# GT-STAR-Lab/MARBLER

Hardware: AMD Instinct MI355X
Metric: env agent-steps/sec (higher is better)
Workload: dtype f32

## Files before the change

marbler_amd/csrc/probes/diag.h:

```cpp
#pragma once

#ifndef RG_CHUNK
#define RG_CHUNK 5
#endif
#ifndef RG_MAX_WAVES
#define RG_MAX_WAVES 1024
#endif
#ifndef RG_TPE_W4
#define RG_TPE_W4 3
#endif
#ifndef RG_TPE_W5
#define RG_TPE_W5 0
#endif
#ifndef RG_TPE_W78
#define RG_TPE_W78 1
#endif
#ifndef RG_TPE_NO_W3
#define RG_TPE_WAVES_ATTR(n) __attribute__((amdgpu_waves_per_eu(n)))
#else
#define RG_TPE_WAVES_ATTR(n)
#endif

namespace rg {
#ifdef RG_STAMPS
constexpr bool kStampsBuild = true;
#else
constexpr bool kStampsBuild = false;
#endif
#ifdef RG_HOST_SIM
constexpr bool kHostSim = true;
#else
constexpr bool kHostSim = false;
#endif
#ifdef RG_TPE_GUARD
constexpr bool kTpeGuard = true;
#else
constexpr bool kTpeGuard = false;
#endif
}

#ifdef RG_STAMPS
#define RG_STAMPS_BEGIN()                                                    \
    const unsigned long long t_start = __builtin_amdgcn_s_memtime();         \
    int stamps[8] = {0, 0, 0, 0, 0, 0, 0, 0};                                \
    RG_STAMPS_CLOCK_BEGIN()
#define RG_STAMP_ALWAYS_5() stamps[5] = static_cast<int>(__builtin_amdgcn_s_memtime() - t_start)
#define RG_PIN1(a) asm volatile("" ::"v"(a))
#define RG_PIN2(a, b) asm volatile("" ::"v"(a), "v"(b))
#define RG_PIN3(a, b, c) asm volatile("" ::"v"(a), "v"(b), "v"(c))
#define RG_PIN4(a, b, c, d) asm volatile("" ::"v"(a), "v"(b), "v"(c), "v"(d))
#define RG_PIN5(a, b, c, d, e) asm volatile("" ::"v"(a), "v"(b), "v"(c), "v"(d), "v"(e))
#ifdef RG_STAMPS_EPI
#define RG_STAMP(i) \
    if ((i) > 2) stamps[i] = static_cast<int>(__builtin_amdgcn_s_memtime() - t_start)
#define RG_STAMP_E(i) stamps[i] = static_cast<int>(__builtin_amdgcn_s_memtime() - t_start)
#else
#define RG_STAMP(i) stamps[i] = static_cast<int>(__builtin_amdgcn_s_memtime() - t_start)
#define RG_STAMP_E(i)
#endif
#ifdef RG_STAMPS_CLOCK
#define RG_STAMPS_CLOCK_BEGIN() const unsigned long long rt_start = __builtin_amdgcn_s_memrealtime();
#define RG_STAMPS_CLOCK_END() stamps[5] = static_cast<int>(__builtin_amdgcn_s_memrealtime() - rt_start);
#else
#define RG_STAMPS_CLOCK_BEGIN()
#define RG_STAMPS_CLOCK_END()
#endif
#define RG_STAMPS_WRITE(lane_, qp_, e0_, E_, max_sweeps_)                                     \
    RG_STAMPS_CLOCK_END()                                                                     \
    if ((lane_) == 0 && (qp_)) {                                                              \
        stamps[7] = (max_sweeps_);                                                            \
        for (int i_ = 0; i_ < 8; ++i_)                                                        \
            if ((e0_) + i_ < (E_)) (qp_)[(e0_) + i_] = stamps[i_];                            \
    }
#else
#define RG_STAMPS_BEGIN()
#define RG_STAMP_ALWAYS_5()
#define RG_PIN1(a)
#define RG_PIN2(a, b)
#define RG_PIN3(a, b, c)
#define RG_PIN4(a, b, c, d)
#define RG_PIN5(a, b, c, d, e)
#define RG_STAMP(i)
#define RG_STAMP_E(i)
#define RG_STAMPS_WRITE(lane_, qp_, e0_, E_, max_sweeps_)
#endif

#if defined(RG_STAMPS) && defined(RG_STAMPS_CTRL)
#define RG_CTRL_TICKS_PARAM , int *ctrl_ticks = nullptr
#define RG_CTRL_TICKS_ARG , ctrl_ticks
#define RG_CTRL_LOCALS() int ctrl_ticks[5] = {0, 0, 0, 0, 0};
#define RG_CTRL_BEGIN(x, y, c, s)                      \
    asm volatile("" ::"v"(x), "v"(y), "v"(c), "v"(s)); \
    unsigned long long ctrl_t = __builtin_amdgcn_s_memtime();
#define RG_CTRL_TICK(i)                                                     \
    {                                                                       \
        const unsigned long long t_ = __builtin_amdgcn_s_memtime();         \
        ctrl_ticks[i] += static_cast<int>(t_ - ctrl_t);                     \
        ctrl_t = t_;                                                        \
    }
#define RG_CTRL_PIN_ROUNDS(GW_, fx, bp, emax) \
    _Pragma("unroll") for (int r_ = 0; r_ < (GW_) - 1; ++r_) asm volatile("" ::"v"(fx[r_]), "v"(bp[r_]), "v"(emax[r_]));
#define RG_CTRL_PIN2(a, b) asm volatile("" ::"v"(a), "v"(b))
#define RG_CTRL_COUNT_SWEEPS(n) ctrl_ticks[3] += (n)
#define RG_HEADING_SINCOS(th, s, c)                                                   \
    asm volatile("" ::"v"(th));                                                       \
    const unsigned long long t_sc = __builtin_amdgcn_s_memtime();                     \
    sincos_spec(th, s, c);                                                            \
    asm volatile("" ::"v"(s), "v"(c));                                                \
    ctrl_ticks[4] += static_cast<int>(__builtin_amdgcn_s_memtime() - t_sc)
#define RG_CTRL_REPORT()                                                                                        \
    stamps[0] = ctrl_ticks[0];                                                                                  \
    stamps[1] = ctrl_ticks[1];                                                                                  \
    stamps[2] = ctrl_ticks[2] * 100 + ctrl_ticks[3];           \
    stamps[3] = ctrl_ticks[4];
#else
#define RG_CTRL_TICKS_PARAM
#define RG_CTRL_TICKS_ARG
#define RG_CTRL_LOCALS()
#define RG_CTRL_BEGIN(x, y, c, s)
#define RG_CTRL_TICK(i)
#define RG_CTRL_PIN_ROUNDS(GW_, fx, bp, emax)
#define RG_CTRL_PIN2(a, b)
#define RG_CTRL_COUNT_SWEEPS(n)
#define RG_HEADING_SINCOS(th, s, c) sincos_spec(th, s, c)
#define RG_CTRL_REPORT()
#endif

#if defined(RG_STAMPS) && defined(RG_STAMPS_CHUNK)
#define RG_CHUNK_LOCALS() int chunk_ticks[4] = {0, 0, 0, 0};
#define RG_CHUNK_DENSE_BEGIN() const unsigned long long t_dense0 = __builtin_amdgcn_s_memtime();
#define RG_CHUNK_DENSE_END(dmin)                                          \
    asm volatile("" ::"v"(dmin));                                         \
    const unsigned long long t_dense1 = __builtin_amdgcn_s_memtime();     \
    chunk_ticks[0] += static_cast<int>(t_dense1 - t_dense0);              \
    chunk_ticks[2] += 1;
#define RG_CHUNK_REPLAY_END(rx, ry)                                                    \
    asm volatile("" ::"v"(rx), "v"(ry));                                               \
    chunk_ticks[1] += static_cast<int>(__builtin_amdgcn_s_memtime() - t_dense1);       \
    chunk_ticks[3] += 1;
#define RG_CHUNK_REPORT()           \
    stamps[0] = chunk_ticks[0];     \
    stamps[1] = chunk_ticks[1];     \
    stamps[2] = chunk_ticks[2] * 1000 + chunk_ticks[3];
#else
#define RG_CHUNK_LOCALS()
#define RG_CHUNK_DENSE_BEGIN()
#define RG_CHUNK_DENSE_END(dmin)
#define RG_CHUNK_REPLAY_END(rx, ry)
#define RG_CHUNK_REPORT()
#endif

#if defined(RG_STAMPS) && !defined(RG_STAMPS_EPI)
#define RG_TSTAMP_MAIN(i) RG_STAMP(i)
#define RG_TSTAMP_EPI(i)
#define RG_TSTAMP_PERIOD(it0) \
    if ((it0) == 0) RG_STAMP(2)
#elif defined(RG_STAMPS)
#define RG_TSTAMP_MAIN(i)
#define RG_TSTAMP_EPI(i) RG_STAMP_E(i)
#define RG_TSTAMP_PERIOD(it0) \
    if ((it0) != 0) RG_STAMP_E(2)
#else
#define RG_TSTAMP_MAIN(i)
#define RG_TSTAMP_EPI(i)
#define RG_TSTAMP_PERIOD(it0)
#endif
#ifdef RG_STAMPS
#define RG_PIN_ARR1(N_, a) _Pragma("unroll") for (int i_ = 0; i_ < (N_); ++i_) asm volatile("" ::"v"(a[i_]))
#define RG_PIN_ARR2(N_, a, b) _Pragma("unroll") for (int i_ = 0; i_ < (N_); ++i_) asm volatile("" ::"v"(a[i_]), "v"(b[i_]))
#define RG_PIN_ARR3(N_, a, b, c) _Pragma("unroll") for (int i_ = 0; i_ < (N_); ++i_) asm volatile("" ::"v"(a[i_]), "v"(b[i_]), "v"(c[i_]))
#define RG_PIN_ARR5(N_, a, b, c, d, e) \
    _Pragma("unroll") for (int i_ = 0; i_ < (N_); ++i_) asm volatile("" ::"v"(a[i_]), "v"(b[i_]), "v"(c[i_]), "v"(d[i_]), "v"(e[i_]))
#else
#define RG_PIN_ARR1(N_, a)
#define RG_PIN_ARR2(N_, a, b)
#define RG_PIN_ARR3(N_, a, b, c)
#define RG_PIN_ARR5(N_, a, b, c, d, e)
#endif
#ifdef RG_TPE_DIAG
#define RG_TPE_DIAG_LOCALS() int diag = 0;
#define RG_TPE_DIAG_SWEEPS(sw, it0) diag |= (sw) << ((it0) == 0 ? 8 : 0)
#define RG_TPE_DIAG_REPLAY(it0, j0, CH_) diag |= 1 << (16 + ((it0) ? 3 : 0) + (j0) / (CH_))
#define RG_TPE_DIAG_REPORT(max_sweeps) max_sweeps = diag
#else
#define RG_TPE_DIAG_LOCALS()
#define RG_TPE_DIAG_SWEEPS(sw, it0)
#define RG_TPE_DIAG_REPLAY(it0, j0, CH_)
#define RG_TPE_DIAG_REPORT(max_sweeps)
#endif
#ifdef RG_TPE_GUARD
#define RG_GUARDED(dst, lo, hi, code, stmt) \
    if ((dst) < (lo) || (dst) >= (hi)) atomicOr(sg.flag, (code)); else { stmt; }
#else
#define RG_GUARDED(dst, lo, hi, code, stmt) stmt
#endif

#ifdef RG_IPM_STAMPS
namespace rg { namespace ipm { __device__ unsigned long long ipm_ticks[8]; } }
#define RG_IPM_T0() unsigned long long ipm_t_ = __builtin_amdgcn_s_memtime();
#define RG_IPM_TICK(i)                                                                              \
    {                                                                                               \
        const unsigned long long t2_ = __builtin_amdgcn_s_memtime();                                \
        if (threadIdx.x == 0 && blockIdx.x == 0) rg::ipm::ipm_ticks[i] += t2_ - ipm_t_;             \
        ipm_t_ = t2_;                                                                               \
    }
#else
#define RG_IPM_T0()
#define RG_IPM_TICK(i)
#endif
```

marbler_amd/csrc/step_group.h:

```cpp
#pragma once
#include <hip/hip_runtime.h>
#include <stdint.h>

#include <type_traits>

#include "device_common.h"
#include "ipm_qp.h"
#include "lidar.h"
#include "team.h"
#include "probes/diag.h"

namespace rg {

__device__ __forceinline__ void out_store4(float *p, float a, float b, float c, float d) {
    *reinterpret_cast<float4 *>(p) = make_float4(a, b, c, d);
}
__device__ __forceinline__ void out_store1(float *p, float a) {
    *p = a;
}

constexpr int CHUNK = RG_CHUNK;
static_assert(CHUNK >= 1 && CHUNK <= 5, "the sparse collision pre-test covers sub-steps 0..2 and 3..4 of a chunk: longer chunks would go untested");

template <int GW, int QPM = 0, typename QpLds = void, bool SPAN = false>
__device__ __forceinline__ int controller(const rg_scenario_params &p, const Consts &k, int N, int ag, bool lane_ok,
                                          bool upd, float x, float y, float c, float s, float gx, float gy, float &v,
                                          float &w, QpLds *qp RG_CTRL_TICKS_PARAM) {
    RG_CTRL_BEGIN(x, y, c, s)
    const float xix = x + k.pd * c, xiy = y + k.pd * s;
    float ux = gx - xix, uy = gy - xiy;
    {
        const float nrm = norm2_spec(ux, uy);
        const float sc = k.pvl / nrm;
        const bool clip = nrm > k.pvl;
        ux = clip ? ux * sc : ux;
        uy = clip ? uy * sc : uy;
    }
    if constexpr (QPM == RG_QP_CVXOPT) {
        {
            const float n2u = ux * ux + uy * uy;
            const bool clip = n2u > k.bml * k.bml;
            if (__any(clip)) {
                const float sc = k.bml / __builtin_sqrtf(n2u);
                ux = clip ? ux * sc : ux;
                uy = clip ? uy * sc : uy;
            }
        }
        const int lane_ = threadIdx.x;
        qp->rec[lane_] = make_float4(xix, xiy, ux, uy);
        __syncthreads();
        int iters = 0;
        if (upd) iters = ipm::solve_qp_n<GW>(N, ipm::make_consts(p), qp->rec + (lane_ & ~(GW - 1)), qp->ws[lane_ / GW], ag);
        __syncthreads();
        const float4 r = qp->rec[lane_];
        ux = r.z;
        uy = r.w;
        RG_CTRL_TICK(1);
        float vv = c * ux + s * uy;
        float ww = k.inv_pd * (-s * ux + c * uy);
        ww = ww > k.wlim ? k.wlim : ww;
        ww = ww < -k.wlim ? -k.wlim : ww;
        vv = vv > k.vmax ? k.vmax : vv;
        vv = vv < -k.vmax ? -k.vmax : vv;
        ww = ww > k.wmax ? k.wmax : ww;
        ww = ww < -k.wmax ? -k.wmax : ww;
        v = upd ? vv : v;
        w = upd ? ww : w;
        RG_CTRL_TICK(2);
        return iters;
    }
    const float bgain = p.barrier_gain, ugain = p.unsafe_barrier_gain, qp_rtol = p.qp_rtol;
    const int qp_cap = p.qp_max_sweeps;
    const bool has_unsafe = p.barrier_has_unsafe_gain != 0;
    float ex[GW - 1], ey[GW - 1], fx[GW - 1], fy[GW - 1], bp[GW - 1], emax[GW - 1];
    float mu[GW - 1], dmu[GW - 1];
    auto pair_consts = [&](float pxi, float pyi, int K, int i) {
        const float dx = xix - pxi, dy = xiy - pyi;
        const float ee = dx * dx + dy * dy;
        const float h = ee - k.r2;
        const float gain = ((h >= 0.0f) | !has_unsafe) ? bgain : ugain;
        const float b = gain * ((h * h) * h);
        const float n2 = 2.0f * ee;
        const bool ok = lane_ok & ((ag ^ K) < N) & (n2 > 0.0f);
        const float rn2 = ok ? 1.0f / n2 : 0.0f;
        ex[i] = dx;
        ey[i] = dy;
        fx[i] = dx * rn2;
        fy[i] = dy * rn2;
        bp[i] = (0.5f * b) * rn2;
        emax[i] = ok ? fmaxf(__builtin_fabsf(dx), __builtin_fabsf(dy)) : 0.0f;
    };
    const bool helper = SPAN && (threadIdx.x & GW) != 0;
    if constexpr (SPAN) {
        static_assert(GW == 8, "16-lane rows of two 8-lane halves");
        const float mx = mirror_upper_half(xix), my = mirror_upper_half(xiy);
        static_for<0, 4>([&](auto SS) {
            constexpr int S = decltype(SS)::value;
            const int K = helper ? S ^ 7 : S;
            if constexpr (S == 0) pair_consts(mx, my, K, 6);
            else pair_consts(xor_lane<S>(mx), xor_lane<S>(my), K, (S ^ 7) - 1);
        });
        static_for<1, 4>([&](auto SS) {
            constexpr int S = decltype(SS)::value, J = (S ^ 7) - 1;
            ex[S - 1] = ex[J];
            ey[S - 1] = ey[J];
            fx[S - 1] = fx[J];
            fy[S - 1] = fy[J];
            bp[S - 1] = bp[J];
            emax[S - 1] = emax[J];
        });
        static_for<3, 7>([&](auto JJ) {
            constexpr int J = decltype(JJ)::value;
            ex[J] = to_lower_half(ex[J]);
            ey[J] = to_lower_half(ey[J]);
            fx[J] = to_lower_half(fx[J]);
            fy[J] = to_lower_half(fy[J]);
            bp[J] = to_lower_half(bp[J]);
            emax[J] = to_lower_half(emax[J]);
        });
    } else {
        static_for<1, GW>([&](auto KK) {
            constexpr int K = decltype(KK)::value;
            pair_consts(xor_lane<K>(xix), xor_lane<K>(xiy), K, K - 1);
        });
    }
    static_for<0, GW - 1>([&](auto KK) { mu[decltype(KK)::value] = dmu[decltype(KK)::value] = 0.0f; });
    RG_CTRL_PIN_ROUNDS(GW, fx, bp, emax)
    RG_CTRL_TICK(0);
    {
        const float n2u = ux * ux + uy * uy;
        const bool clip = n2u > k.bml * k.bml;
        if (__any(clip)) {
            const float sc = k.bml / __builtin_sqrtf(n2u);
            ux = clip ? ux * sc : ux;
            uy = clip ? uy * sc : uy;
        }
    }
    const float uhx = ux, uhy = uy;
    bool active = upd & !helper;
    int sweeps = 0, my_sweeps = 0;
    auto sweep = [&](auto PH) {
        constexpr int PHASE = decltype(PH)::value;
        ++sweeps;
        if (active) {
            float chg = 0.0f, pa = 0.0f, pb = 0.0f;
            static_for<1, GW>([&](auto KK) {
                constexpr int K = decltype(KK)::value;
                const float pux = xor_lane<K>(ux), puy = xor_lane<K>(uy);
                const float c0 = mu[K - 1] - bp[K - 1];
                const float t = __builtin_fmaf(fy[K - 1], puy - uy, c0);
                float mn = __builtin_fmaf(fx[K - 1], pux - ux, t);
                mn = (mn > 0.0f) ? mn : 0.0f;
                const float delta = mn - mu[K - 1];
                mu[K - 1] = mn;
                ux = __builtin_fmaf(delta, ex[K - 1], ux);
                uy = __builtin_fmaf(delta, ey[K - 1], uy);
                chg = fmaxf(chg, __builtin_fabsf(delta) * emax[K - 1]);
                if constexpr (PHASE == 2) dmu[K - 1] = delta;
                if constexpr (PHASE == 3) {
                    const float dd = delta - dmu[K - 1];
                    pa = __builtin_fmaf(dd, delta, pa);
                    pb = __builtin_fmaf(dd, dd, pb);
                    dmu[K - 1] = delta;
                }
            });
            my_sweeps = sweeps;
            const float um = lane_ok ? fmaxf(__builtin_fabsf(ux), __builtin_fabsf(uy)) : 0.0f;
            const float gchg = group_max_nonneg<GW>(chg);
            const float gum = fmaxf(k.bml, group_max_nonneg<GW>(um));
            active = (gchg > qp_rtol * gum) & (sweeps < qp_cap);
            if constexpr (PHASE == 3) {
                if (active) {
                    const float ga = group_sum<GW>(pa), gb = group_sum<GW>(pb);
                    const bool ok = (gb > 0.0f) & (ga < 0.0f) & (-ga < 32.0f * gb);
                    const float gam = ok ? ga / gb : 0.0f;
                    float sx = uhx, sy = uhy;
                    static_for<1, GW>([&](auto KK) {
                        constexpr int K = decltype(KK)::value;
                        float m = __builtin_fmaf(-gam, dmu[K - 1], mu[K - 1]);
                        m = (m > 0.0f) ? m : 0.0f;
                        mu[K - 1] = m;
                        sx = __builtin_fmaf(m, ex[K - 1], sx);
                        sy = __builtin_fmaf(m, ey[K - 1], sy);
                    });
                    ux = sx;
                    uy = sy;
                }
            }
        }
    };
    while (__any(active)) {
        sweep(std::integral_constant<int, 1>{});
        if (!__any(active)) break;
        sweep(std::integral_constant<int, 2>{});
        if (!__any(active)) break;
        sweep(std::integral_constant<int, 3>{});
        if (!__any(active)) break;
        sweep(std::integral_constant<int, 0>{});
    }
    if constexpr (SPAN) {
        ux = to_upper_half(ux);
        uy = to_upper_half(uy);
    }
    RG_CTRL_PIN2(ux, uy);
    RG_CTRL_TICK(1);
    float vv = c * ux + s * uy;
    float ww = k.inv_pd * (-s * ux + c * uy);
    ww = ww > k.wlim ? k.wlim : ww;
    ww = ww < -k.wlim ? -k.wlim : ww;
    vv = vv > k.vmax ? k.vmax : vv;
    vv = vv < -k.vmax ? -k.vmax : vv;
    ww = ww > k.wmax ? k.wmax : ww;
    ww = ww < -k.wmax ? -k.wmax : ww;
    v = upd ? vv : v;
    w = upd ? ww : w;
    RG_CTRL_PIN2(v, w);
    RG_CTRL_COUNT_SWEEPS(sweeps);
    RG_CTRL_TICK(2);
    return my_sweeps;
}

template <int GW, int OD, int NT>
__device__ __forceinline__ void write_neighbour_obs(Lds<GW> &lds, int N, int Knb, int ag, int gbase, bool lane_ok,
                                                    float x, float y, float *obs_row) {
    constexpr int M = NT > 0 ? NT - 1 : GW - 1;
    unsigned long long key[M > 0 ? M : 1];
    bool ok[M > 0 ? M : 1];
    int rank[M > 0 ? M : 1], who[M > 0 ? M : 1];
    static_for<0, M>([&](auto RR) {
        constexpr int r = decltype(RR)::value;
        int j = ag + r + 1;
        j = j >= N ? j - N : j;
        j = j & (GW - 1);
        who[r] = j;
        const float2 pxy = *reinterpret_cast<const float2 *>(&lds.own[gbase + j][0]);
        const float dx = pxy.x - x, dy = pxy.y - y;
        const float d2 = dx * dx + dy * dy;
        ok[r] = lane_ok & (r + 1 < N);
        const unsigned int hi = ok[r] ? __builtin_bit_cast(unsigned int, d2) : 0xFFFFFFFFu;
        key[r] = (static_cast<unsigned long long>(hi) << 32) | static_cast<unsigned int>(j);
        rank[r] = M - 1 - r;
    });
    const bool all_others = Knb >= N - 1;
    static_for<1, M>([&](auto KK) {
        constexpr int k = decltype(KK)::value;
        static_for<0, k>([&](auto QQ) {
            constexpr int q = decltype(QQ)::value;
            const int q_first = key[q] < key[k] ? 1 : 0;
            rank[k] += q_first;
            rank[q] -= q_first;
        });
    });
    float row[M > 0 ? M : 1][OD];
    static_for<0, M>([&](auto RR) {
        constexpr int r = decltype(RR)::value;
        const float *src = &lds.own[gbase + who[r]][0];
        if constexpr (OD == 4) {
            const float4 v = *reinterpret_cast<const float4 *>(src);
            row[r][0] = v.x;
            row[r][1] = v.y;
            row[r][2] = v.z;
            row[r][3] = v.w;
        } else {
#pragma unroll
            for (int c = 0; c < OD; ++c) row[r][c] = src[c];
        }
    });
    static_for<0, M>([&](auto RR) {
        constexpr int r = decltype(RR)::value;
        const int j = who[r];
        const int slot = all_others ? (j < ag ? j : j - 1) : rank[r];
        if (ok[r] & (all_others | (slot < Knb))) {
            float *o = obs_row + (slot + 1) * OD;
            if constexpr (OD == 4) {
                out_store4(o, row[r][0], row[r][1], row[r][2], row[r][3]);
            } else {
#pragma unroll
                for (int c = 0; c < OD; ++c) o[c] = row[r][c];
            }
        }
    });
}

template <int SCN, int GW, bool OBS_ONLY, int NT, bool AHEAD, bool GYM, int QPM = 0, typename QpLds = void, typename Sync = WgSync,
          bool LIDAR = false, bool TEAM = false, bool SPAN = false>
__device__ __forceinline__ void step_once(const KernelArgs &a, Lds<GW> &lds, const StepView &sv, QpLds *qp_lds = nullptr,
                                          const rg_lidar_params *lid = nullptr, const rg_team_params *tm = nullptr) {
    static_assert(!SPAN || (GW == 8 && QPM == 0 && !GYM && !LIDAR && !TEAM), "the 16-lane rows: exact mode, GW = 8, no side blocks");
    constexpr int RW = SPAN ? 2 * GW : GW;
    constexpr int EPW = WAVE / RW;
    RG_STAMPS_BEGIN()
    const rg_scenario_params &p = a.p;
    const Consts &k = a.k;
    const float *q_poses = a.st.poses, *q_carry = a.st.carry_dist, *q_ret = a.st.ep_return, *q_sum = a.st.done_return_sum;
    const int32_t *q_steps = a.st.episode_steps, *q_act = sv.actions, *q_cnt = a.st.done_count, *q_stp = a.st.done_steps_sum;
    int32_t *q_el = GYM ? sv.io.elapsed : nullptr;
    const int q_tl = GYM ? sv.io.time_limit : 0;
    const int32_t *q_rc = a.st.reset_count, *q_nep = AHEAD ? a.st.next_episode : nullptr;
    const float *q_nin = AHEAD ? a.st.next_init : nullptr;
    const int q_nst = AHEAD ? a.next_stride : 0;
    const int q_E = a.E, q_epw = a.envs_per_wave, q_P = p.num_prey, q_N = p.n_agents, q_G = gridDim.x;
    asm volatile("" ::"s"(q_poses), "s"(q_carry), "s"(q_ret), "s"(q_sum), "s"(q_steps), "s"(q_act), "s"(q_cnt), "s"(q_stp),
                 "s"(q_E), "s"(q_epw), "s"(q_P), "s"(q_N), "s"(q_G), "s"(q_rc));
    if constexpr (GYM) asm volatile("" ::"s"(q_el), "s"(q_tl));
    if constexpr (AHEAD) asm volatile("" ::"s"(q_nep), "s"(q_nin), "s"(q_nst));
    const float *q_prey = a.st.prey_loc;
    const uint8_t *q_sen = a.st.prey_sensed, *q_cap = a.st.prey_captured, *q_loaded = a.st.loaded, *q_grid = a.st.grid;
    const uint8_t *q_pix = a.st.pixel_type, *q_reached = a.st.reached_goal;
    const int32_t *q_gcol = a.st.goal_col, *q_msg = a.st.messages, *q_zone = a.st.zone_load, *q_load = a.st.load;
    if constexpr (SCN == RG_SCN_PREDATOR_CAPTURE_PREY) asm volatile("" ::"s"(q_prey), "s"(q_sen), "s"(q_cap));
    else if constexpr (SCN == RG_SCN_WAREHOUSE) asm volatile("" ::"s"(q_loaded));
    else if constexpr (SCN == RG_SCN_SIMPLE) asm volatile("" ::"s"(q_prey));
    else if constexpr (SCN == RG_SCN_ARCTIC_TRANSPORT) asm volatile("" ::"s"(q_grid), "s"(q_pix), "s"(q_reached), "s"(q_gcol));
    else asm volatile("" ::"s"(q_msg), "s"(q_zone), "s"(q_load));
    int32_t *q_tidx = TEAM ? tm->team_index : nullptr;
    const float *q_tstep = TEAM ? tm->agent_step : nullptr, *q_tsr = TEAM ? tm->sensing_radius : nullptr;
    const float *q_tcr = TEAM ? tm->capture_radius : nullptr;
    const int32_t *q_ttq = TEAM ? tm->torque : nullptr;
    const int q_tC = TEAM ? tm->n_sets : 1;
    if constexpr (TEAM) {
        asm volatile("" ::"s"(q_tidx), "s"(q_tstep), "s"(q_tC));
        if constexpr (SCN == RG_SCN_PREDATOR_CAPTURE_PREY) asm volatile("" ::"s"(q_tsr), "s"(q_tcr));
        else if constexpr (SCN == RG_SCN_MATERIAL_TRANSPORT) asm volatile("" ::"s"(q_ttq));
    }

    const int N = NT > 0 ? NT : q_N;
    const int lane = threadIdx.x;
    const int ag = lane & (GW - 1);
    const int g = lane / RW;
    const int gbase = lane & ~(RW - 1);
    const bool helper = SPAN && (lane & GW) != 0;
    const int epw = q_epw > 0 ? q_epw : EPW;
    const int chunk = xcd_chunk(q_G);
    const int e = chunk * epw + g;
    const bool env_ok = (g < epw) & (e < q_E);
    const bool lane_ok = env_ok && ag < N;
    const bool env_st = env_ok & !helper, lane_st = lane_ok & !helper;
    const size_t eN = static_cast<size_t>(e) * N;

#define RG_LATE(v) asm volatile("" : "+v"(v))
    float x = 0.0f, y = 0.0f, th = 0.0f, carry = 0.0f;
    int act = 4;
    int steps_raw = 0;
    float agent_step = 0.0f, sr = 0.0f, cr = 0.0f;
    float st_ret = 0.0f, st_sum = 0.0f;
    int st_cnt = 0, st_steps = 0;
    const bool stats = (!OBS_ONLY) && q_ret != nullptr;
    int pix = 0, reached = 0;
    int team_raw = 0, tq_raw = 0;
    if constexpr (TEAM) {
        if (env_ok) team_raw = q_tidx[e];
    }
    if (lane_ok) {
        const float *X = q_poses + eN * 3;
        x = X[ag];
        y = X[N + ag];
        th = X[2 * N + ag];
        if constexpr (!OBS_ONLY) act = q_act[eN + ag];
        if constexpr (SCN == RG_SCN_ARCTIC_TRANSPORT) pix = q_pix[eN + ag];
        if constexpr (!TEAM) {
        agent_step = p.agent_step[ag];
        if constexpr (SCN == RG_SCN_PREDATOR_CAPTURE_PREY) {
            sr = p.sensing_radius[ag];
            cr = p.capture_radius[ag];
        }
        }
        if constexpr (!OBS_ONLY) carry = q_carry[eN + ag];
        if constexpr (TEAM) {
            const size_t ti = static_cast<size_t>(team_clamp(team_raw, q_tC)) * N + ag;
            agent_step = q_tstep[ti];
            if constexpr (SCN == RG_SCN_PREDATOR_CAPTURE_PREY) {
                sr = q_tsr[ti];
                cr = q_tcr[ti];
            }
            if constexpr (SCN == RG_SCN_MATERIAL_TRANSPORT) tq_raw = q_ttq[ti];
        }
    }
    int rc_raw = -1;
    const bool ahead = AHEAD && (!OBS_ONLY) && q_nst > 0 && a.auto_reset;
    int nx_tag = -2;
    float nx_pose[3] = {0.0f, 0.0f, 0.0f};
    float nx_a = 0.0f, nx_b = 0.0f;
    uint32_t nx_grid[7] = {0, 0, 0, 0, 0, 0, 0};
    auto load_next = [&](bool want) {
        if (want) {
            const float *nb = q_nin + static_cast<size_t>(e) * q_nst;
            if (ag < N) {
                nx_pose[0] = nb[ag];
                nx_pose[1] = nb[N + ag];
                nx_pose[2] = nb[2 * N + ag];
            }
            if constexpr (SCN == RG_SCN_PREDATOR_CAPTURE_PREY || SCN == RG_SCN_SIMPLE) {
                if (ag < q_P) {
                    nx_a = nb[3 * N + 2 * ag];
                    nx_b = nb[3 * N + 2 * ag + 1];
                }
            } else if constexpr (SCN == RG_SCN_MATERIAL_TRANSPORT) {
                if (ag < 2) nx_a = nb[3 * N + ag];
            } else if constexpr (SCN == RG_SCN_ARCTIC_TRANSPORT) {
                const uint32_t *gb = reinterpret_cast<const uint32_t *>(nb + 3 * N);
#pragma unroll
                for (int t = 0; t < 6; ++t) nx_grid[t] = gb[ag * 6 + t];
                nx_grid[6] = gb[24];
            }
        }
    };
    int el_raw = 0;
    if (env_ok) {
        steps_raw = q_steps[e];
        if (!OBS_ONLY && a.auto_reset) rc_raw = q_rc[e];
        if constexpr (GYM) el_raw = q_el[e];
        if (ahead) nx_tag = q_nep[e];
        if (stats && ag == 0) {
            st_ret = q_ret[e];
            st_sum = q_sum[e];
            st_cnt = q_cnt[e];
            st_steps = q_stp[e];
        }
    }
    uint32_t sen_lo = 0, sen_hi = 0, cap_lo = 0, cap_hi = 0;
    int flag_raw[4] = {0, 0, 0, 0};
    int loaded = 0;
    float goal_x = 0.0f, goal_y = 0.0f;
    uint32_t grid_pre[6] = {0, 0, 0, 0, 0, 0};
    int goal_col = 1;
    int load = 0, zone0 = 0, zone1 = 0;
    int msg[4] = {0, 0, 0, 0};
    float2 prey_r[8];
#pragma unroll
    for (int t = 0; t < 8; ++t) prey_r[t] = make_float2(0.0f, 0.0f);
    static_assert(SCN != RG_SCN_ARCTIC_TRANSPORT || GW == 4, "ArcticTransport is a 4-agent scenario");
    if constexpr (SCN == RG_SCN_PREDATOR_CAPTURE_PREY) {
        const int P = q_P;
        if (P <= 8) {
            if (env_ok) {
                const float2 *src = reinterpret_cast<const float2 *>(q_prey) + static_cast<size_t>(e) * P;
#pragma unroll
                for (int t = 0; t < 8; ++t) prey_r[t] = src[t < P ? t : P - 1];
                if (ag < P) {
                    flag_raw[0] = q_sen[static_cast<size_t>(e) * P + ag];
                    flag_raw[1] = q_cap[static_cast<size_t>(e) * P + ag];
                }
                if constexpr (GW < 8)
                    if (ag + GW < P) {
                        flag_raw[2] = q_sen[static_cast<size_t>(e) * P + ag + GW];
                        flag_raw[3] = q_cap[static_cast<size_t>(e) * P + ag + GW];
                    }
            }
        } else {
            if (env_ok) {
                for (int i = ag; i < 2 * P; i += GW) lds.prey[g][i] = q_prey[static_cast<size_t>(e) * 2 * P + i];
                for (int i = ag; i < P; i += GW) {
                    const uint32_t sb = q_sen[static_cast<size_t>(e) * P + i] != 0;
                    const uint32_t cb = q_cap[static_cast<size_t>(e) * P + i] != 0;
                    if (i < 32) {
                        sen_lo |= sb << i;
                        cap_lo |= cb << i;
                    } else {
                        sen_hi |= sb << (i - 32);
                        cap_hi |= cb << (i - 32);
                    }
                }
            }
            sen_lo = group_or<GW>(sen_lo);
            cap_lo = group_or<GW>(cap_lo);
            if (P > 32) {
                sen_hi = group_or<GW>(sen_hi);
                cap_hi = group_or<GW>(cap_hi);
            }
        }
    } else if constexpr (SCN == RG_SCN_WAREHOUSE) {
        if (lane_ok) loaded = q_loaded[eN + ag];
    } else if constexpr (SCN == RG_SCN_SIMPLE) {
        if (env_ok) {
            goal_x = q_prey[static_cast<size_t>(e) * 2];
            goal_y = q_prey[static_cast<size_t>(e) * 2 + 1];
        }
    } else if constexpr (SCN == RG_SCN_ARCTIC_TRANSPORT) {
        if (env_ok) {
            const uint32_t *gsrc = reinterpret_cast<const uint32_t *>(q_grid + static_cast<size_t>(e) * 96);
#pragma unroll
            for (int t = 0; t < 6; ++t) grid_pre[t] = gsrc[ag * 6 + t];
            goal_col = q_gcol[e];
        }
        if (lane_ok) reached = q_reached[eN + ag];
    } else {
        if (env_ok) {
#pragma unroll
            for (int i = 0; i < 4; ++i) {
                if (OBS_ONLY || i >= N) msg[i] = q_msg[4 * e + i];
                else msg[i] = q_act[eN + i];
            }
            zone0 = q_zone[2 * e];
            zone1 = q_zone[2 * e + 1];
        }
        if (lane_ok) load = q_load[eN + ag];
    }

    int viol = 0, max_sweeps = 0;
    bool replayed = false;
    float dist = 0.0f;
    if constexpr (!OBS_ONLY) {
        RG_PIN5(x, y, th, carry, act);
        RG_STAMP(0);
        float gx = x, gy = y;
        {
            const int mv = (SCN == RG_SCN_MATERIAL_TRANSPORT) ? act / 4 : act;
            float sd = agent_step;
            if constexpr (SCN == RG_SCN_ARCTIC_TRANSPORT) {
                const float nrm_s = p.arctic_normal_step, slow_s = p.arctic_slow_step, fast_s = p.arctic_fast_step;
                const float water = pix == 1 ? slow_s : pix == 2 ? fast_s : nrm_s;
                const float ice = pix == 1 ? fast_s : pix == 2 ? slow_s : nrm_s;
                sd = ag < 2 ? fast_s : ag == 3 ? water : ice;
            }
            const float cgx = clamp_spec(gx, p.left, p.right), cgy = clamp_spec(gy, p.up, p.down);
            const float lft = (gx - sd) > p.left ? (gx - sd) : p.left;
            const float rgt = (gx + sd) < p.right ? (gx + sd) : p.right;
            const float upw = (gy - sd) > p.up ? (gy - sd) : p.up;
            const float dwn = (gy + sd) < p.down ? (gy + sd) : p.down;
            gx = mv == 0 ? lft : mv == 1 ? rgt : cgx;
            gy = mv == 2 ? upw : mv == 3 ? dwn : cgy;
        }
        const int thr_pre = __builtin_bit_cast(int, k.thr_pre);
        const int ghost_q = __builtin_bit_cast(int, __builtin_amdgcn_cvt_pkrtz(1000.0f + 32.0f * ag, -1000.0f));
        float v = 0.0f, w = 0.0f, s = 0.0f, c = 1.0f;
        RG_CHUNK_LOCALS()
        RG_CTRL_LOCALS()
        float acc = carry, last = 0.0f;
        bool dead = false;
        float fin_x = 0.0f, fin_y = 0.0f;
        float bx = x, by = y, ox = 0.0f, oy = 0.0f;
        const bool penalize = p.penalize_violations != 0;
        const int U = p.update_frequency, period = p.controller_period;
        for (int it0 = 0; it0 < U; it0 += period) {
            const int n = (U - it0) < period ? (U - it0) : period;
            RG_HEADING_SINCOS(th, s, c);
            const int sw = controller<GW, QPM, QpLds, SPAN>(p, k, N, ag, lane_ok, env_ok & !dead, x, y, c, s, gx, gy, v, w, qp_lds RG_CTRL_TICKS_ARG);
            max_sweeps = sw > max_sweeps ? sw : max_sweeps;
            const float dtv = k.dt * v, dtw = k.dt * w;
            float sd, cd;
            sincos_small_spec(dtw, sd, cd);
            if (__any(__builtin_fabsf(dtw) > 0.25f)) {
                float sd2, cd2;
                sincos_spec(dtw, sd2, cd2);
                const bool big = __builtin_fabsf(dtw) > 0.25f;
                sd = big ? sd2 : sd;
                cd = big ? cd2 : cd;
            }
            if (it0 == 0) RG_STAMP(1);
            const float mrg = __builtin_fmaf((CHUNK - 1) * 1.000001f, __builtin_fabsf(dtv), PRE_SLACK);
            int n_exec = n;
            bool died_now = false;
            const float mstep = lane_ok ? __builtin_fmaf(__builtin_fabsf(k.coll_off), __builtin_fabsf(dtw), __builtin_fabsf(dtv)) * 1.00001f : 0.0f;
            const float M2 = 2.0f * group_max_nonneg<GW>(mstep);
            auto thr_span = [&](int span) {
                const float t = (k.lin_pre + PRE_SLACK) + static_cast<float>(span) * M2;
                return __builtin_bit_cast(int, (t * t) * 1.00002f);
            };
            const int thr_s1 = thr_span(1), thr_s2 = thr_span(2);
            const bool sparse_ok = (k.lin_pre + 2.0f * M2) < 0.24f;

            auto run_chunk = [&](auto CC, int j0) {
                constexpr int C = decltype(CC)::value;
                const float x0 = x, y0 = y, ox0 = ox, oy0 = oy, c0 = c, s0 = s;
                const bool live = lane_ok & !dead;
                int q[C];
                const bool bnd_any = live & ((__builtin_fabsf(x - k.xc) + mrg > k.xh) | (__builtin_fabsf(y - k.yc) + mrg > k.yh));
                static_for<0, C>([&](auto UU) {
                    constexpr int u = decltype(UU)::value;
                    const float fx = __builtin_fmaf(k.coll_off, c, x), fy = __builtin_fmaf(k.coll_off, s, y);
                    const int qr = __builtin_bit_cast(int, __builtin_amdgcn_cvt_pkrtz(fx, fy));
                    q[u] = live ? qr : ghost_q;
                    ox = __builtin_fmaf(c, dtv, ox);
                    oy = __builtin_fmaf(s, dtv, oy);
                    x = bx + ox;
                    y = by + oy;
                    const float cn = __builtin_fmaf(c, cd, -(s * sd));
                    const float sn = __builtin_fmaf(s, cd, c * sd);
                    c = cn;
                    s = sn;
                });
                auto pair_min = [&](int qv) {
                    constexpr bool QUAD_COVER = GW == 8 && NT >= 5 && NT <= 7;
                    constexpr int R = QUAD_COVER ? NT - 1 : GW - 1;
                    int d[R];
                    auto diff = [&](int partner_q) {
                        return __builtin_bit_cast(int, __builtin_bit_cast(half2v, qv) - __builtin_bit_cast(half2v, partner_q));
                    };
                    if constexpr (QUAD_COVER) {
                        static_for<1, 4>([&](auto KK) { d[decltype(KK)::value - 1] = diff(xor_lane_i<decltype(KK)::value>(qv)); });
                        static_for<0, NT - 4>([&](auto MM) { d[3 + decltype(MM)::value] = diff(cross_lane_i<decltype(MM)::value>(qv)); });
                    } else {
                        static_for<1, GW>([&](auto KK) { d[decltype(KK)::value - 1] = diff(xor_lane_i<decltype(KK)::value>(qv)); });
                    }
                    int dm = 0x7FFFFFFF;
                    dot2_batch<R>(d);
#pragma unroll
                    for (int r = 0; r < R; ++r) dm = d[r] < dm ? d[r] : dm;
                    return dm;
                };
                int dmin_u[C];
                bool sparse_hit = live & !sparse_ok;
                {
                    constexpr int SPAN0 = C - 1 < 2 ? C - 1 : 2;
                    const int t0 = SPAN0 == 0 ? thr_pre : SPAN0 == 1 ? thr_s1 : thr_s2;
                    if constexpr (SPAN && C >= 4) {
                        const int t3 = C == 4 ? thr_pre : thr_s1;
                        const int dm = pair_min(helper ? q[3] : q[0]);
                        sparse_hit = sparse_hit | (dm <= (helper ? t3 : t0));
                        dmin_u[0] = dmin_u[3] = dm;
                    } else {
                        dmin_u[0] = pair_min(q[0]);
                        sparse_hit = sparse_hit | (dmin_u[0] <= t0);
                        if constexpr (C >= 4) {
                            const int t3 = C == 4 ? thr_pre : thr_s1;
                            dmin_u[3] = pair_min(q[3]);
                            sparse_hit = sparse_hit | (dmin_u[3] <= t3);
                        }
                    }
                }
                if (penalize && __any(sparse_hit | bnd_any)) {
                RG_CHUNK_DENSE_BEGIN()
                if constexpr (SPAN && C >= 4) {
                    const int mine = dmin_u[0], other = xor_lane_i<8>(mine);
                    dmin_u[0] = helper ? other : mine;
                    dmin_u[3] = helper ? mine : other;
                }
                if constexpr (SPAN && C >= 3) {
                    const int mine = pair_min(helper ? q[2] : q[1]), other = xor_lane_i<8>(mine);
                    if constexpr (C == 5) dmin_u[4] = pair_min(q[4]);
                    dmin_u[1] = helper ? other : mine;
                    dmin_u[2] = helper ? mine : other;
                } else {
                    static_for<1, C>([&](auto UU) {
                        constexpr int u = decltype(UU)::value;
                        if constexpr (u != 3) dmin_u[u] = pair_min(q[u]);
                    });
                }
                int dmin = dmin_u[0];
                static_for<1, C>([&](auto UU) { dmin = dmin_u[decltype(UU)::value] < dmin ? dmin_u[decltype(UU)::value] : dmin; });
                RG_CHUNK_DENSE_END(dmin)
                if (__any((dmin <= thr_pre) | bnd_any)) {
                    replayed = true;
                    float rx = x0, ry = y0, rox = ox0, roy = oy0, rc = c0, rs = s0;
                    static_for<0, C>([&](auto UU) {
                        constexpr int u = decltype(UU)::value;
                        const bool bnd = lane_ok & !dead & ((rx < k.xmin) | (rx > k.xmax) | (ry < k.ymin) | (ry > k.ymax));
                        const float fx = __builtin_fmaf(k.coll_off, rc, rx), fy = __builtin_fmaf(k.coll_off, rs, ry);
                        bool col = false;
                        if (!__any(dmin_u[u] <= thr_pre)) {
                        } else if constexpr (GW == 8 && NT >= 5 && NT <= 7) {
                            static_for<1, 4>([&](auto KK) {
                                constexpr int K = decltype(KK)::value;
                                const float dx = fx - xor_lane<K>(fx), dy = fy - xor_lane<K>(fy);
                                col = col | (((ag ^ K) < N) & (dx * dx + dy * dy <= k.coll_lim2));
                            });
                            static_for<0, NT - 4>([&](auto MM) {
                                constexpr int M = decltype(MM)::value;
                                const float dx = fx - cross_lane<M>(fx), dy = fy - cross_lane<M>(fy);
                                col = col | (dx * dx + dy * dy <= k.coll_lim2);
                            });
                        } else {
                            static_for<1, GW>([&](auto KK) {
                                constexpr int K = decltype(KK)::value;
                                const float dx = fx - xor_lane<K>(fx), dy = fy - xor_lane<K>(fy);
                                col = col | (((ag ^ K) < N) & (dx * dx + dy * dy <= k.coll_lim2));
                            });
                        }
                        col = col & lane_ok & !dead;
                        const int code = (group_any<GW>(col, gbase) ? 1 : 0) | (group_any<GW>(bnd, gbase) ? 2 : 0);
                        rox = __builtin_fmaf(rc, dtv, rox);
                        roy = __builtin_fmaf(rs, dtv, roy);
                        rx = bx + rox;
                        ry = by + roy;
                        if (env_ok & !dead & (code != 0)) {
                            viol = code;
                            n_exec = j0 + u + 1;
                            died_now = true;
                            dead = true;
                            fin_x = rx;
                            fin_y = ry;
                        }
                        const float cn = __builtin_fmaf(rc, cd, -(rs * sd));
                        const float sn = __builtin_fmaf(rs, cd, rc * sd);
                        rc = cn;
                        rs = sn;
                    });
                    RG_CHUNK_REPLAY_END(rx, ry)
                }
                }
            };
            int j = 0;
            for (; j + CHUNK <= n; j += CHUNK) run_chunk(std::integral_constant<int, CHUNK>{}, j);
            static_for<1, CHUNK>([&](auto RR) {
                if (n - j == decltype(RR)::value) run_chunk(RR, j);
            });

            const bool upd = env_ok & (!dead | died_now);
            const float ne = static_cast<float>(n_exec);
            const float adv = __builtin_fabsf(dtv);
            th = upd ? wrap_spec(__builtin_fmaf(ne, dtw, th)) : th;
            acc = upd ? __builtin_fmaf(ne, adv, acc) : acc;
            last = upd ? adv : last;
            {
                const float tx = x - bx, ty = y - by;
                ox = (bx - (x - tx)) + (ox - tx);
                oy = (by - (y - ty)) + (oy - ty);
                bx = x;
                by = y;
            }
            if (it0 == 0) RG_STAMP(2);
            if (!__any(env_ok & !dead)) break;
        }
        if (dead) {
            x = fin_x;
            y = fin_y;
        }
        dist = viol ? acc : acc - last;
        carry = last;
        RG_STAMP(3);
        RG_CTRL_REPORT()
        RG_CHUNK_REPORT()
    }

    const int D = p.obs_dim;
    float *obs_row = sv.io.obs + (eN + ag) * D;
    bool done = false;
    int remaining = -1;
    float reward = 0.0f;
    RG_LATE(steps_raw);
    const int steps = steps_raw + (OBS_ONLY ? 0 : 1);
    RG_LATE(rc_raw);
    RG_LATE(nx_tag);
    const bool have_next = ahead & (nx_tag == rc_raw);
    const bool next_early = env_ok & have_next & ((viol != 0) | (steps > p.max_episode_steps));
    if constexpr (AHEAD) load_next(next_early & !helper);

    if constexpr (SCN == RG_SCN_PREDATOR_CAPTURE_PREY) {
        const int P = q_P;
        if constexpr (TEAM) {
            RG_LATE(sr);
            RG_LATE(cr);
        }
        const float sr2 = sr * sr, cr2 = cr * cr;
        if (P > 8) Sync::sync();
        if (P <= 8) {
            RG_LATE(flag_raw[0]);
            RG_LATE(flag_raw[1]);
            uint32_t sb = (flag_raw[0] != 0 ? 1u : 0u) << ag, cb = (flag_raw[1] != 0 ? 1u : 0u) << ag;
            if constexpr (GW < 8) {
                RG_LATE(flag_raw[2]);
                RG_LATE(flag_raw[3]);
                sb |= (flag_raw[2] != 0 ? 1u : 0u) << (ag + GW);
                cb |= (flag_raw[3] != 0 ? 1u : 0u) << (ag + GW);
            }
            sen_lo = group_or<GW>(sb);
            cap_lo = group_or<GW>(cb);
        }
        uint32_t nsen_lo = sen_lo, nsen_hi = sen_hi, ncap_lo = cap_lo, ncap_hi = cap_hi;
        auto scan = [&](int lo, int hi, auto &&f) {
            for (int i0 = lo; i0 < hi; i0 += 4) {
                float2 pl[4];
#pragma unroll
                for (int t = 0; t < 4; ++t) {
                    const int i = (i0 + t) < hi ? (i0 + t) : (hi - 1);
                    pl[t] = *reinterpret_cast<const float2 *>(&lds.prey[g][2 * i]);
                }
#pragma unroll
                for (int t = 0; t < 4; ++t) {
                    const float dx = x - pl[t].x, dy = y - pl[t].y;
                    f(i0 + t, (i0 + t) < hi, pl[t].x, pl[t].y, dx * dx + dy * dy);
                }
            }
        };
        float closest = -1.0f, qx = -5.0f, qy = -5.0f;
        if (P <= 8) {
            const float2 (&pl)[8] = prey_r;
            float d2[8];
            uint32_t s_b = 0, c_b = 0;
            const bool acts = lane_ok & (act == 4);
#pragma unroll
            for (int t = 0; t < 8; ++t) {
                const float dx = x - pl[t].x, dy = y - pl[t].y;
                d2[t] = dx * dx + dy * dy;
                const bool in = t < P;
                s_b |= ((in & lane_ok & (d2[t] <= sr2)) ? 1u : 0u) << t;
                c_b |= ((in & acts & (d2[t] <= cr2)) ? 1u : 0u) << t;
            }
            if constexpr (!OBS_ONLY) {
                s_b = group_or<GW>(s_b);
                c_b = group_or<GW>(c_b);
                nsen_lo = sen_lo | (s_b & ~cap_lo);
                ncap_lo = cap_lo | (nsen_lo & c_b & ~cap_lo);
                if (env_st && ag < P) {
                    a.st.prey_sensed[static_cast<size_t>(e) * P + ag] = (nsen_lo >> ag) & 1u;
                    a.st.prey_captured[static_cast<size_t>(e) * P + ag] = (ncap_lo >> ag) & 1u;
                }
                if constexpr (GW < 8)
                    if (env_ok && ag + GW < P) {
                        a.st.prey_sensed[static_cast<size_t>(e) * P + ag + GW] = (nsen_lo >> (ag + GW)) & 1u;
                        a.st.prey_captured[static_cast<size_t>(e) * P + ag + GW] = (ncap_lo >> (ag + GW)) & 1u;
                    }
            }
#pragma unroll
            for (int t = 0; t < 8; ++t) {
                const bool cap = ((ncap_lo >> t) & 1u) != 0;
                const bool take = (t < P) & !cap & (d2[t] <= sr2) & ((d2[t] < closest) | (closest == -1.0f));
                qx = take ? pl[t].x : qx;
                qy = take ? pl[t].y : qy;
                closest = take ? d2[t] : closest;
            }
        } else {
        if constexpr (!OBS_ONLY) {
            uint32_t s_lo = 0, s_hi = 0, c_lo = 0, c_hi = 0;
            const bool acts = lane_ok & (act == 4);
            const int P32 = P < 32 ? P : 32;
            scan(0, P32, [&](int i, bool in, float, float, float d2) {
                s_lo |= ((in & lane_ok & (d2 <= sr2)) ? 1u : 0u) << (i & 31);
                c_lo |= ((in & acts & (d2 <= cr2)) ? 1u : 0u) << (i & 31);
            });
            s_lo = group_or<GW>(s_lo);
            c_lo = group_or<GW>(c_lo);
            nsen_lo = sen_lo | (s_lo & ~cap_lo);
            ncap_lo = cap_lo | (nsen_lo & c_lo & ~cap_lo);
            if (P > 32) {
                scan(32, P, [&](int i, bool in, float, float, float d2) {
                    s_hi |= ((in & lane_ok & (d2 <= sr2)) ? 1u : 0u) << ((i - 32) & 31);
                    c_hi |= ((in & acts & (d2 <= cr2)) ? 1u : 0u) << ((i - 32) & 31);
                });
                s_hi = group_or<GW>(s_hi);
                c_hi = group_or<GW>(c_hi);
                nsen_hi = sen_hi | (s_hi & ~cap_hi);
                ncap_hi = cap_hi | (nsen_hi & c_hi & ~cap_hi);
            }
            if (env_st) {
                for (int i = ag; i < P; i += GW) {
                    const uint32_t sw_ = i < 32 ? nsen_lo >> i : nsen_hi >> (i - 32);
                    const uint32_t cw_ = i < 32 ? ncap_lo >> i : ncap_hi >> (i - 32);
                    a.st.prey_sensed[static_cast<size_t>(e) * P + i] = sw_ & 1u;
                    a.st.prey_captured[static_cast<size_t>(e) * P + i] = cw_ & 1u;
                }
            }
        }
        {
            auto nearest = [&](uint32_t capmask, int base) {
                return [&, capmask, base](int i, bool in, float px, float py, float d2) {
                    const bool cap = ((capmask >> ((i - base) & 31)) & 1u) != 0;
                    const bool take = in & !cap & (d2 <= sr2) & ((d2 < closest) | (closest == -1.0f));
                    qx = take ? px : qx;
                    qy = take ? py : qy;
                    closest = take ? d2 : closest;
                };
            };
            scan(0, P < 32 ? P : 32, nearest(ncap_lo, 0));
            if (P > 32) scan(32, P, nearest(ncap_hi, 32));
        }
        }
        RG_STAMP_E(0);
        const int od = p.capability_aware ? 6 : 4;
        lds.own[lane][0] = x;
        lds.own[lane][1] = y;
        lds.own[lane][2] = qx;
        lds.own[lane][3] = qy;
        lds.own[lane][4] = sr;
        lds.own[lane][5] = cr;
        Sync::sync();
        if (od == 6) {
            if (lane_st) {
#pragma unroll
                for (int cc = 0; cc < 6; ++cc) obs_row[cc] = lds.own[lane][cc];
            }
            write_neighbour_obs<GW, 6, NT>(lds, N, p.num_neighbors, ag, gbase, lane_st, x, y, obs_row);
        } else {
            if (lane_st) out_store4(obs_row, x, y, qx, qy);
            write_neighbour_obs<GW, 4, NT>(lds, N, p.num_neighbors, ag, gbase, lane_st, x, y, obs_row);
        }
        RG_STAMP_E(1);
        if constexpr (!OBS_ONLY) {
            const int unseen0 = P - __builtin_popcount(sen_lo) - __builtin_popcount(sen_hi);
            const int left0 = P - __builtin_popcount(cap_lo) - __builtin_popcount(cap_hi);
            const int unseen1 = P - __builtin_popcount(nsen_lo) - __builtin_popcount(nsen_hi);
            const int left1 = P - __builtin_popcount(ncap_lo) - __builtin_popcount(ncap_hi);
            if (viol) {
                reward = p.violation_reward;
                done = true;
            } else {
                reward = 0.0f;
                reward = reward + static_cast<float>(unseen0 - unseen1) * p.sense_reward;
                reward = reward + static_cast<float>(left0 - left1) * p.capture_reward;
                reward = reward + p.time_penalty;
                if (steps > p.max_episode_steps || left1 == 0) {
                    done = true;
                    remaining = left1;
                }
            }
        }
    } else if constexpr (SCN == RG_SCN_WAREHOUSE) {
        lds.own[lane][0] = x;
        lds.own[lane][1] = y;
        lds.own[lane][2] = loaded ? 1.0f : 0.0f;
        Sync::sync();
        if (lane_st) {
            obs_row[0] = x;
            obs_row[1] = y;
            obs_row[2] = loaded ? 1.0f : 0.0f;
        }
        write_neighbour_obs<GW, 3, NT>(lds, N, p.num_neighbors, ag, gbase, lane_st, x, y, obs_row);
        if constexpr (!OBS_ONLY) {
            if (viol) {
                reward = p.violation_reward;
                done = true;
            } else {
                const bool green = (ag % 2) == 0;
                if (loaded) {
                    if (x < -1.5f + p.goal_width && ((green && y > 0.0f) || (!green && y <= 0.0f))) {
                        reward = p.unload_reward;
                        loaded = 0;
                    }
                } else {
                    if (x > 1.5f - p.goal_width && ((!green && y > 0.0f) || (green && y <= 0.0f))) {
                        reward = p.load_reward;
                        loaded = 1;
                    }
                }
                done = steps > p.max_episode_steps;
                if (lane_st) a.st.loaded[eN + ag] = static_cast<uint8_t>(loaded);
            }
        }
    } else if constexpr (SCN == RG_SCN_SIMPLE) {
        lds.own[lane][0] = x;
        lds.own[lane][1] = y;
        Sync::sync();
        if (lane_st) {
            obs_row[0] = x;
            obs_row[1] = y;
            obs_row[2 * N] = goal_x;
            obs_row[2 * N + 1] = goal_y;
        }
        write_neighbour_obs<GW, 2, NT>(lds, N, N - 1, ag, gbase, lane_st, x, y, obs_row);
        if constexpr (!OBS_ONLY) {
            if (viol) {
                reward = p.violation_reward;
                done = true;
            } else {
                const float dx = x - goal_x, dy = y - goal_y;
                const float r = -(dx * dx + dy * dy);
                reward = r * p.reward_scaler;
                done = steps > p.max_episode_steps;
            }
        }
    } else if constexpr (SCN == RG_SCN_ARCTIC_TRANSPORT) {
        {
            uint32_t *gdst = reinterpret_cast<uint32_t *>(&lds.grid[g][0]);
#pragma unroll
            for (int t = 0; t < 6; ++t) gdst[ag * 6 + t] = grid_pre[t];
        }
        Sync::sync();
        const uint8_t *grid = &lds.grid[g][0];
        int row = -static_cast<int>((y - 1.0f) / 0.25f), col = static_cast<int>((x + 1.5f) / 0.25f);
        row = row < 0 ? 0 : row > 7 ? 7 : row;
        col = col < 0 ? 0 : col > 11 ? 11 : col;
        if constexpr (!OBS_ONLY) {
            pix = grid[row * 12 + col];
            reached = reached | (pix == 3 ? 1 : 0);
        }
        const int here = grid[row * 12 + col];
        lds.own[lane][0] = x;
        lds.own[lane][1] = y;
        lds.own[lane][2] = static_cast<float>(here);
        lds.aload[lane] = row * 16 + col;
        Sync::sync();
        const float goalx = static_cast<float>(goal_col) * 0.25f - 1.5f, goaly = -1.0f * 0.25f + 0.75f;
        if (lane_ok) {
            obs_row[0] = x;
            obs_row[1] = y;
            obs_row[2] = static_cast<float>(here);
            const int o0 = ag == 0 ? 1 : ag == 1 ? 0 : ag == 2 ? 3 : 2;
            const int o1 = ag < 2 ? 2 : 0, o2 = ag < 2 ? 3 : 1;
            const int oth[3] = {o0, o1, o2};
#pragma unroll
            for (int m = 0; m < 3; ++m) {
                obs_row[3 + 3 * m + 0] = lds.own[gbase + oth[m]][0];
                obs_row[3 + 3 * m + 1] = lds.own[gbase + oth[m]][1];
                obs_row[3 + 3 * m + 2] = lds.own[gbase + oth[m]][2];
            }
            obs_row[12] = goalx;
            obs_row[13] = goaly;
#pragma unroll
            for (int i = 0; i < 2; ++i) {
                const int rc = lds.aload[gbase + i];
                const int r_ = rc >> 4, c_ = rc & 15;
                const int left = c_ > 0 ? c_ - 1 : c_, right = c_ < 11 ? c_ + 1 : c_;
                const int up = r_ > 0 ? r_ - 1 : r_, down = r_ < 7 ? r_ + 1 : r_;
                float *o = obs_row + 14 + 8 * i;
                o[0] = static_cast<float>(grid[up * 12 + left]);
                o[1] = static_cast<float>(grid[r_ * 12 + left]);
                o[2] = static_cast<float>(grid[down * 12 + left]);
                o[3] = static_cast<float>(grid[up * 12 + c_]);
                o[4] = static_cast<float>(grid[down * 12 + c_]);
                o[5] = static_cast<float>(grid[up * 12 + right]);
                o[6] = static_cast<float>(grid[r_ * 12 + right]);
                o[7] = static_cast<float>(grid[down * 12 + right]);
            }
        }
        if constexpr (LIDAR) write_lidar<SCN, GW, OBS_ONLY, Sync>(*lid, a, lds, lane, gbase, N, ag, lane_ok, x, y, th, obs_row);
        if constexpr (!OBS_ONLY) {
            const float dx = x - goalx, dy = y - goaly;
            lds.ax[lane] = dx * dx + dy * dy;
            lds.ay[lane] = static_cast<float>(pix * 2 + reached);
            Sync::sync();
            if (viol) {
                reward = p.violation_reward;
                done = true;
            } else {
                reward = 0.0f;
                bool all_reached = true;
#pragma unroll
                for (int j = 2; j < 4; ++j) {
                    const int pr = static_cast<int>(lds.ay[gbase + j]);
                    const bool rj = (pr & 1) != 0;
                    if (!rj) reward = reward + p.not_reached_penalty;
                    if ((pr >> 1) != 3) reward = reward + p.dist_multiplier * lds.ax[gbase + j];
                    all_reached = all_reached && rj;
                }
                done = steps > p.max_episode_steps;
                if (!done) done = all_reached;
            }
            if (lane_ok) {
                a.st.pixel_type[eN + ag] = static_cast<uint8_t>(pix);
                a.st.reached_goal[eN + ag] = static_cast<uint8_t>(reached);
            }
        }
    } else {
#pragma unroll
        for (int i = 0; i < 4; ++i) {
            RG_LATE(msg[i]);
            if (!OBS_ONLY && i < N) msg[i] = msg[i] % 4;
        }
        if constexpr (TEAM) RG_LATE(tq_raw);
        if (lane_st) {
            obs_row[0] = x;
            obs_row[1] = y;
            obs_row[2] = static_cast<float>(load);
            obs_row[3] = static_cast<float>(zone0);
            obs_row[4] = static_cast<float>(zone1);
#pragma unroll
            for (int i = 0; i < 4; ++i) obs_row[5 + i] = static_cast<float>(msg[i]);
            if (p.capability_aware) {
                if constexpr (TEAM) obs_row[9] = static_cast<float>(tq_raw);
                else obs_row[9] = static_cast<float>(p.torque[ag]);
                obs_row[10] = agent_step;
            }
        }
        if constexpr (!OBS_ONLY) {
            lds.ax[lane] = x;
            lds.ay[lane] = y;
            lds.aload[lane] = load;
            if constexpr (TEAM) team_lds<SCN, GW>().torque[lane] = tq_raw;
            Sync::sync();
            if (viol) {
                reward = p.violation_reward;
                done = true;
            } else {
                reward = p.time_penalty;
                const float egw = p.end_goal_width;
                const float zr2 = p.zone1_radius * p.zone1_radius;
                bool any_load = false;
                for (int j = 0; j < N; ++j) {
                    const float jx = lds.ax[gbase + j], jy = lds.ay[gbase + j];
                    int jl = lds.aload[gbase + j];
                    int tq;
                    if constexpr (TEAM) tq = team_lds<SCN, GW>().torque[gbase + j];
                    else tq = p.torque[j];
                    if (jl > 0) {
                        if (jx < -1.5f + egw) {
                            reward = reward + static_cast<float>(jl) * p.unload_multiplier;
                            jl = 0;
                        }
                    } else {
                        if (jx > 1.5f - egw) {
                            if (zone1 > tq) {
                                jl = tq;
                                zone1 -= tq;
                            } else {
                                jl = zone1;
                                zone1 = 0;
                            }
                            reward = reward + static_cast<float>(jl) * p.load_multiplier;
                        } else if (jx * jx + jy * jy <= zr2) {
                            if (zone0 > tq) {
                                jl = tq;
                                zone0 -= tq;
                            } else {
                                jl = zone0;
                                zone0 = 0;
                            }
                            reward = reward + static_cast<float>(jl) * p.load_multiplier;
                        }
                    }
                    if (j == ag) load = jl;
                    any_load = any_load || (jl != 0);
                }
                done = steps > p.max_episode_steps;
                if (!done) done = (zone0 == 0 && zone1 == 0 && !any_load);
            }
            int total = 0;
            {
                lds.aload[lane] = lane_ok ? load : 0;
                Sync::sync();
                for (int j = 0; j < N; ++j) total += lds.aload[gbase + j];
            }
            if (done) remaining = zone0 + zone1 + total;
            if (lane_st) a.st.load[eN + ag] = load;
            if (lane_st && ag == 0) {
                a.st.zone_load[2 * e] = zone0;
                a.st.zone_load[2 * e + 1] = zone1;
            }
            if (lane_st && ag < 4) a.st.messages[4 * e + ag] = msg[ag == 0 ? 0 : ag == 1 ? 1 : ag == 2 ? 2 : 3];
        }
    }

    if constexpr (LIDAR && SCN != RG_SCN_ARCTIC_TRANSPORT) write_lidar<SCN, GW, OBS_ONLY, Sync>(*lid, a, lds, lane, gbase, N, ag, lane_ok, x, y, th, obs_row);
    RG_STAMP(4);
    if constexpr (!OBS_ONLY) {
        constexpr bool gym = GYM;
        bool trunc = false;
        if (gym) {
            RG_LATE(el_raw);
            trunc = env_ok & !done & (el_raw + 1 >= q_tl);
        }
        const bool ended = done | trunc;
        float rsum = 0.0f;
        if ((stats && !p.shared_reward) || gym) {
            Sync::sync();
            lds.ax[lane] = lane_ok ? reward : 0.0f;
            Sync::sync();
            for (int j = 0; j < N; ++j) rsum = rsum + lds.ax[gbase + j];
        }
        if (lane_st) {
            float *X = a.st.poses + eN * 3;
            X[ag] = x;
            X[N + ag] = y;
            X[2 * N + ag] = th;
            a.st.carry_dist[eN + ag] = carry;
            out_store1(sv.io.reward + eN + ag, reward);
            out_store1(sv.io.dist_travelled + eN + ag, dist);
            if (ag == 0) {
                a.st.episode_steps[e] = steps;
                if (stats) {
                    RG_LATE(st_ret);
                    RG_LATE(st_sum);
                    RG_LATE(st_cnt);
                    RG_LATE(st_steps);
                    float ret = st_ret + (p.shared_reward ? reward : rsum);
                    if (ended) {
                        a.st.done_return_sum[e] = st_sum + ret;
                        a.st.done_count[e] = st_cnt + 1;
                        a.st.done_steps_sum[e] = st_steps + steps;
                        ret = 0.0f;
                    }
                    a.st.ep_return[e] = ret;
                }
                sv.io.done[e] = done ? 1 : 0;
                if (gym) {
                    q_el[e] = ended ? 0 : el_raw + 1;
                    sv.io.truncated[e] = trunc ? 1 : 0;
                    sv.io.ended[e] = ended ? 1 : 0;
                    sv.io.reward_sum[e] = rsum;
                }
                sv.io.violation[e] = static_cast<uint8_t>(viol);
                sv.io.remaining[e] = remaining;
                if (sv.io.qp_sweeps) sv.io.qp_sweeps[e] = max_sweeps;
            }
            if constexpr (GYM) {
                if (sv.io.zero_obs_on_end && ended) {
                    for (int c = 0; c < D; ++c) obs_row[c] = 0.0f;
                }
            }
        }
        RG_STAMP(5);
        if (a.auto_reset && __any(env_ok & ended)) {
            Sync::sync();
            if constexpr (AHEAD) load_next(env_st & ended & have_next & !next_early);
            if (__any(env_ok & ended & !have_next)) reset_group<SCN, GW, Sync>(a, lds, e, g, ag, env_st & ended & !have_next, rc_raw);
            if (env_st & ended & have_next) {
                if (ag < N) {
                    float *X = a.st.poses + eN * 3;
                    X[ag] = nx_pose[0];
                    X[N + ag] = nx_pose[1];
                    X[2 * N + ag] = nx_pose[2];
                    a.st.carry_dist[eN + ag] = 0.0f;
                    if constexpr (SCN == RG_SCN_WAREHOUSE) a.st.loaded[eN + ag] = 0;
                    if constexpr (SCN == RG_SCN_MATERIAL_TRANSPORT) {
                        a.st.load[eN + ag] = 0;
                        if (ag < 4) a.st.messages[4 * e + ag] = 0;
                    }
                    if constexpr (SCN == RG_SCN_ARCTIC_TRANSPORT) {
                        a.st.pixel_type[eN + ag] = 0;
                        a.st.reached_goal[eN + ag] = 0;
                    }
                }
                if constexpr (SCN == RG_SCN_PREDATOR_CAPTURE_PREY || SCN == RG_SCN_SIMPLE) {
                    const int P = q_P;
                    const float *nb = q_nin + static_cast<size_t>(e) * q_nst + 3 * N;
                    for (int i = ag; i < P; i += GW) {
                        float *pl = a.st.prey_loc + (static_cast<size_t>(e) * P + i) * 2;
                        pl[0] = i == ag ? nx_a : nb[2 * i];
                        pl[1] = i == ag ? nx_b : nb[2 * i + 1];
                        if constexpr (SCN == RG_SCN_PREDATOR_CAPTURE_PREY) {
                            a.st.prey_sensed[static_cast<size_t>(e) * P + i] = 0;
                            a.st.prey_captured[static_cast<size_t>(e) * P + i] = 0;
                        }
                    }
                } else if constexpr (SCN == RG_SCN_MATERIAL_TRANSPORT) {
                    if (ag < 2) a.st.zone_load[2 * e + ag] = __builtin_bit_cast(int32_t, nx_a);
                } else if constexpr (SCN == RG_SCN_ARCTIC_TRANSPORT) {
                    uint32_t *gd = reinterpret_cast<uint32_t *>(a.st.grid + static_cast<size_t>(e) * 96);
#pragma unroll
                    for (int t = 0; t < 6; ++t) gd[ag * 6 + t] = nx_grid[t];
                    if (ag == 0) a.st.goal_col[e] = static_cast<int32_t>(nx_grid[6]);
                }
                if (ag == 0) {
                    a.st.reset_count[e] = rc_raw + 1;
                    a.st.episode_steps[e] = 0;
                }
            }
            if constexpr (TEAM) {
                if (env_ok & ended & (ag == 0)) q_tidx[e] = team_draw(*tm, static_cast<uint64_t>(a.env_offset + e), rc_raw, a.seed);
            }
        }
        if (AHEAD && ahead && !(replayed | __any(max_sweeps > 2)) && __any(env_ok & !ended & !have_next)) {
            const bool need = env_st & !ended & !have_next;
            Sync::sync();
            reset_group<SCN, GW, Sync>(a, lds, e, g, ag, need, rc_raw, reset_dst_next(a, e));
            if (need && ag == 0) a.st.next_episode[e] = rc_raw;
        }
        RG_STAMP(6);
        RG_STAMPS_WRITE(lane, sv.io.qp_sweeps, chunk * EPW, a.E, max_sweeps)
    }
}

template <int SCN, int GW, bool OBS_ONLY, int NT, bool ROLLOUT, bool GYM, int QPM, bool SPAN>
__device__ __forceinline__ void step_kernel_body(const KernelArgs &a) {
    __shared__ Lds<GW> lds;
    const int N = NT > 0 ? NT : a.p.n_agents;
    if constexpr (QPM == RG_QP_CVXOPT) {
        static_assert(GW == 4 || GW == 8, "the interior-point mode admits n_agents <= 8");
        __shared__ ipm::GroupLds<GW> qp_lds;
        if constexpr (!ROLLOUT) {
            step_once<SCN, GW, OBS_ONLY, NT, true, GYM, QPM>(a, lds, step_view(a, 0, N, a.p.obs_dim), &qp_lds);
        } else {
            for (int t = 0; t < a.num_steps; ++t) {
                if (t) __syncthreads();
                step_once<SCN, GW, OBS_ONLY, NT, false, false, QPM>(a, lds, step_view(a, t, N, a.p.obs_dim), &qp_lds);
            }
        }
    } else if constexpr (SPAN) {
        static_assert(!ROLLOUT && !OBS_ONLY, "the 16-lane rows: the single-step launch");
        step_once<SCN, GW, false, NT, true, GYM, QPM, void, WgSync, false, false, true>(a, lds, step_view(a, 0, N, a.p.obs_dim));
    } else if constexpr (!ROLLOUT) {
        step_once<SCN, GW, OBS_ONLY, NT, true, GYM, QPM>(a, lds, step_view(a, 0, N, a.p.obs_dim), static_cast<void *>(nullptr));
    } else {
        for (int t = 0; t < a.num_steps; ++t) {
            if (t) __syncthreads();
            step_once<SCN, GW, OBS_ONLY, NT, false, false, QPM>(a, lds, step_view(a, t, N, a.p.obs_dim), static_cast<void *>(nullptr));
        }
    }
}

template <int SCN, int GW, bool OBS_ONLY, int NT, bool ROLLOUT, bool GYM = false, int QPM = 0>
__global__ __launch_bounds__(WAVE) void step_kernel(const KernelArgs a) {
    step_kernel_body<SCN, GW, OBS_ONLY, NT, ROLLOUT, GYM, QPM, false>(a);
}
template <int SCN, int GW, bool OBS_ONLY, int NT, bool ROLLOUT, int ROW, std::enable_if_t<ROW == 16, int> = 0>
__global__ __launch_bounds__(WAVE) void step_kernel(const KernelArgs a) {
    step_kernel_body<SCN, GW, OBS_ONLY, NT, ROLLOUT, false, 0, true>(a);
}

template <int SCN, int GW>
__global__ __launch_bounds__(WAVE) void reset_kernel(const KernelArgs a) {
    constexpr int EPW = WAVE / GW;
    __shared__ Lds<GW> lds;
    const int lane = threadIdx.x;
    const int ag = lane & (GW - 1);
    const int g = lane / GW;
    const int e = blockIdx.x * EPW + g;
    const bool env_ok = e < a.E;
    const bool want = env_ok && (a.reset_mask == nullptr || a.reset_mask[e] != 0);
    if (!__any(want)) return;
    const bool stats = want && ag == 0 && a.st.ep_return != nullptr;
    const int steps_before = stats ? a.st.episode_steps[e] : 0;
    reset_group<SCN, GW>(a, lds, e, g, ag, want);
    if (stats) {
        if ((a.reset_flags & RG_RESET_BOOK_EPISODE) && steps_before > 0) {
            a.st.done_return_sum[e] = a.st.done_return_sum[e] + a.st.ep_return[e];
            a.st.done_count[e] = a.st.done_count[e] + 1;
            a.st.done_steps_sum[e] = a.st.done_steps_sum[e] + steps_before;
        }
        a.st.ep_return[e] = 0.0f;
    }
}

}


namespace rg {

inline int group_width(int N) { return N <= 4 ? 4 : N <= 8 ? 8 : 16; }

template <int SCN, bool OBS_ONLY, bool ROLLOUT>
static hipError_t launch_step_scn(const KernelArgs &a_in, hipStream_t stream) {
    const int gw = group_width(a_in.p.n_agents);
    KernelArgs a = a_in;
    int epw = WAVE / gw;
    if constexpr (!kStampsBuild) {
        while (epw >= 2 && (a.E + epw / 2 - 1) / (epw / 2) <= RG_MAX_WAVES) epw /= 2;
        a.envs_per_wave = epw;
    }
    const int grid = (a.E + epw - 1) / epw;
    if constexpr (!OBS_ONLY) {
        if (a.p.qp_mode == RG_QP_CVXOPT) return ROLLOUT ? launch_rollout_ipm(a, grid, stream) : launch_step_ipm(a, grid, stream);
    }
    if constexpr (!OBS_ONLY && !ROLLOUT) {
        if (a.io.elapsed) {
            if (gw == 4) hipLaunchKernelGGL((step_kernel<SCN, 4, false, 0, false, true>), dim3(grid), dim3(WAVE), 0, stream, a);
            else if (gw == 16) hipLaunchKernelGGL((step_kernel<SCN, 16, false, 0, false, true>), dim3(grid), dim3(WAVE), 0, stream, a);
            else hipLaunchKernelGGL((step_kernel<SCN, 8, false, 0, false, true>), dim3(grid), dim3(WAVE), 0, stream, a);
            return hipGetLastError();
        }
    }
    if constexpr (!OBS_ONLY && !ROLLOUT && !kStampsBuild) {
        if (a_in.envs_per_wave >= 0 && gw == 8 && epw <= 4) {
            switch (a.p.n_agents) {
                case 5: hipLaunchKernelGGL((step_kernel<SCN, 8, false, 5, false, 16>), dim3(grid), dim3(WAVE), 0, stream, a); break;
                case 6: hipLaunchKernelGGL((step_kernel<SCN, 8, false, 6, false, 16>), dim3(grid), dim3(WAVE), 0, stream, a); break;
                case 7: hipLaunchKernelGGL((step_kernel<SCN, 8, false, 7, false, 16>), dim3(grid), dim3(WAVE), 0, stream, a); break;
                default: hipLaunchKernelGGL((step_kernel<SCN, 8, false, 8, false, 16>), dim3(grid), dim3(WAVE), 0, stream, a); break;
            }
            return hipGetLastError();
        }
    }
    if (gw == 4) hipLaunchKernelGGL((step_kernel<SCN, 4, OBS_ONLY, 0, ROLLOUT>), dim3(grid), dim3(WAVE), 0, stream, a);
    else if (gw == 16) hipLaunchKernelGGL((step_kernel<SCN, 16, OBS_ONLY, 0, ROLLOUT>), dim3(grid), dim3(WAVE), 0, stream, a);
    else if constexpr (OBS_ONLY) hipLaunchKernelGGL((step_kernel<SCN, 8, true, 0, false>), dim3(grid), dim3(WAVE), 0, stream, a);
    else if (a.p.n_agents == 5) hipLaunchKernelGGL((step_kernel<SCN, 8, false, 5, ROLLOUT>), dim3(grid), dim3(WAVE), 0, stream, a);
    else if (a.p.n_agents == 6) hipLaunchKernelGGL((step_kernel<SCN, 8, false, 6, ROLLOUT>), dim3(grid), dim3(WAVE), 0, stream, a);
    else if (a.p.n_agents == 7) hipLaunchKernelGGL((step_kernel<SCN, 8, false, 7, ROLLOUT>), dim3(grid), dim3(WAVE), 0, stream, a);
    else hipLaunchKernelGGL((step_kernel<SCN, 8, false, 8, ROLLOUT>), dim3(grid), dim3(WAVE), 0, stream, a);
    return hipGetLastError();
}

template <bool OBS_ONLY, bool ROLLOUT>
static hipError_t launch_step_group(const KernelArgs &a, hipStream_t stream) {
    static_assert(!(OBS_ONLY && ROLLOUT), "rg_get_obs is a single launch");
    switch (a.p.scenario) {
        case RG_SCN_PREDATOR_CAPTURE_PREY:
            return launch_step_scn<RG_SCN_PREDATOR_CAPTURE_PREY, OBS_ONLY, ROLLOUT>(a, stream);
        case RG_SCN_WAREHOUSE:
            return launch_step_scn<RG_SCN_WAREHOUSE, OBS_ONLY, ROLLOUT>(a, stream);
        case RG_SCN_MATERIAL_TRANSPORT:
            return launch_step_scn<RG_SCN_MATERIAL_TRANSPORT, OBS_ONLY, ROLLOUT>(a, stream);
        case RG_SCN_SIMPLE:
            return launch_step_scn<RG_SCN_SIMPLE, OBS_ONLY, ROLLOUT>(a, stream);
        case RG_SCN_ARCTIC_TRANSPORT:
            if constexpr (!OBS_ONLY) {
                if (a.p.qp_mode == RG_QP_CVXOPT)
                    return ROLLOUT ? launch_rollout_ipm(a, (a.E + 15) / 16, stream) : launch_step_ipm(a, (a.E + 15) / 16, stream);
            }
            if constexpr (!OBS_ONLY && !ROLLOUT) {
                if (a.io.elapsed) {
                    hipLaunchKernelGGL((step_kernel<RG_SCN_ARCTIC_TRANSPORT, 4, false, 0, false, true>), dim3((a.E + 15) / 16),
                                       dim3(WAVE), 0, stream, a);
                    return hipGetLastError();
                }
            }
            hipLaunchKernelGGL((step_kernel<RG_SCN_ARCTIC_TRANSPORT, 4, OBS_ONLY, 0, ROLLOUT>), dim3((a.E + 15) / 16), dim3(WAVE), 0,
                               stream, a);
            return hipGetLastError();
        default:
            return hipErrorInvalidValue;
    }
}

template <int SCN, bool ROLLOUT>
static hipError_t launch_ipm_scn(const KernelArgs &a, int grid, hipStream_t stream) {
    constexpr int Q = RG_QP_CVXOPT;
    const int gw = SCN == RG_SCN_ARCTIC_TRANSPORT ? 4 : group_width(a.p.n_agents);
    if constexpr (!ROLLOUT) {
        if (a.io.elapsed) {
            if (gw == 4) hipLaunchKernelGGL((step_kernel<SCN, 4, false, 0, false, true, Q>), dim3(grid), dim3(WAVE), 0, stream, a);
            else if constexpr (SCN != RG_SCN_ARCTIC_TRANSPORT) hipLaunchKernelGGL((step_kernel<SCN, 8, false, 0, false, true, Q>), dim3(grid), dim3(WAVE), 0, stream, a);
            return hipGetLastError();
        }
    }
    if (gw == 4) hipLaunchKernelGGL((step_kernel<SCN, 4, false, 0, ROLLOUT, false, Q>), dim3(grid), dim3(WAVE), 0, stream, a);
    else if constexpr (SCN != RG_SCN_ARCTIC_TRANSPORT) hipLaunchKernelGGL((step_kernel<SCN, 8, false, 0, ROLLOUT, false, Q>), dim3(grid), dim3(WAVE), 0, stream, a);
    return hipGetLastError();
}
template <bool ROLLOUT>
static hipError_t launch_ipm_group(const KernelArgs &a, int grid, hipStream_t stream) {
    switch (a.p.scenario) {
        case RG_SCN_PREDATOR_CAPTURE_PREY: return launch_ipm_scn<RG_SCN_PREDATOR_CAPTURE_PREY, ROLLOUT>(a, grid, stream);
        case RG_SCN_WAREHOUSE: return launch_ipm_scn<RG_SCN_WAREHOUSE, ROLLOUT>(a, grid, stream);
        case RG_SCN_MATERIAL_TRANSPORT: return launch_ipm_scn<RG_SCN_MATERIAL_TRANSPORT, ROLLOUT>(a, grid, stream);
        case RG_SCN_SIMPLE: return launch_ipm_scn<RG_SCN_SIMPLE, ROLLOUT>(a, grid, stream);
        case RG_SCN_ARCTIC_TRANSPORT: return launch_ipm_scn<RG_SCN_ARCTIC_TRANSPORT, ROLLOUT>(a, grid, stream);
        default: return hipErrorInvalidValue;
    }
}

}
```

Before: 1.639 billion.

## Park epilogue pointers and constants in LDS to relieve scalar registers

Loads the scenario constants and output/state pointers once at kernel start, pins hot scalar values in SGPRs, and packs the epilogue-only pointers and constants into a per-wave LDS word array using v_writelane. The epilogue then reads them back from LDS instead of reloading kernarg/param memory after the long controller loop. The aim is to avoid scalar memory reloads and SGPR spills around the epilogue. In exchange it adds LDS traffic, a wave barrier, and address-space casts, and the inline-asm pinning may raise register pressure.

```diff
diff --git a/marbler_amd/csrc/probes/diag.h b/marbler_amd/csrc/probes/diag.h
--- a/marbler_amd/csrc/probes/diag.h
+++ b/marbler_amd/csrc/probes/diag.h
@@ -150,6 +150,18 @@
 #define RG_CHUNK_REPORT()
 #endif
 
+#ifdef RG_SHADOW_TRIPS
+#define RG_SHADOW_SCALAR_TRIPS()                                                                                          \
+    rg::static_for<0, RG_SHADOW_TRIPS>([&](auto II_) {                                                                    \
+        int t_;                                                                                                           \
+        asm volatile("s_load_dword %0, %1, %2\n\ts_waitcnt lgkmcnt(0)"                                                    \
+                     : "=s"(t_)                                                                                           \
+                     : "s"(__builtin_amdgcn_kernarg_segment_ptr()), "n"(0x298 + 64 * (decltype(II_)::value % 5)));        \
+    });
+#else
+#define RG_SHADOW_SCALAR_TRIPS()
+#endif
+
 #if defined(RG_STAMPS) && !defined(RG_STAMPS_EPI)
 #define RG_TSTAMP_MAIN(i) RG_STAMP(i)
 #define RG_TSTAMP_EPI(i)
diff --git a/marbler_amd/csrc/step_group.h b/marbler_amd/csrc/step_group.h
--- a/marbler_amd/csrc/step_group.h
+++ b/marbler_amd/csrc/step_group.h
@@ -12,18 +12,60 @@
 
 namespace rg {
 
+template <typename T>
+using GlobalPtr = __attribute__((address_space(1))) T *;
 __device__ __forceinline__ void out_store4(float *p, float a, float b, float c, float d) {
     *reinterpret_cast<float4 *>(p) = make_float4(a, b, c, d);
 }
-__device__ __forceinline__ void out_store1(float *p, float a) {
+__device__ __forceinline__ void out_store4(GlobalPtr<float> p, float a, float b, float c, float d) {
+#if defined(__HIP_DEVICE_COMPILE__)
+    *(GlobalPtr<float4>)p = make_float4(a, b, c, d);
+#else
+    out_store4((float *)p, a, b, c, d);
+#endif
+}
+template <typename P>
+__device__ __forceinline__ void out_store1(P p, float a) {
     *p = a;
 }
+
+__device__ __forceinline__ uint32_t *park_lds() {
+    __shared__ uint32_t words[WAVE];
+    return words;
+}
+__device__ __forceinline__ void park_publish() {
+    __builtin_amdgcn_fence(__ATOMIC_RELEASE, "wavefront");
+    __builtin_amdgcn_wave_barrier();
+    __builtin_amdgcn_fence(__ATOMIC_ACQUIRE, "wavefront");
+}
+template <int LANE>
+__device__ __forceinline__ void park_word(int &park, int word) {
+    static_assert(LANE >= 0 && LANE < WAVE, "one word per lane of the wave");
+    asm("v_writelane_b32 %0, %1, %2" : "+v"(park) : "s"(word), "n"(LANE));
+}
+template <int I>
+__device__ __forceinline__ void park_put(int &park, const void *ptr) {
+    const uint64_t b = reinterpret_cast<uint64_t>(ptr);
+    park_word<2 * I>(park, static_cast<int>(b));
+    park_word<2 * I + 1>(park, static_cast<int>(b >> 32));
+}
+template <typename T, int I>
+__device__ __forceinline__ GlobalPtr<T> park_get(const uint32_t *pk) {
+    return (GlobalPtr<T>)((static_cast<uint64_t>(pk[2 * I + 1]) << 32) | pk[2 * I]);
+}
+
+struct StepConsts : Consts {
+    float bgain, ugain, qp_rtol;
+    int qp_cap, has_unsafe;
+    float left, right, up, down;
+    int penalize, U, period;
+};
 
 constexpr int CHUNK = RG_CHUNK;
 static_assert(CHUNK >= 1 && CHUNK <= 5, "the sparse collision pre-test covers sub-steps 0..2 and 3..4 of a chunk: longer chunks would go untested");
 
 template <int GW, int QPM = 0, typename QpLds = void, bool SPAN = false>
-__device__ __forceinline__ int controller(const rg_scenario_params &p, const Consts &k, int N, int ag, bool lane_ok,
+__device__ __forceinline__ int controller(const rg_scenario_params &p, const StepConsts &k, int N, int ag, bool lane_ok,
                                           bool upd, float x, float y, float c, float s, float gx, float gy, float &v,
                                           float &w, QpLds *qp RG_CTRL_TICKS_PARAM) {
     RG_CTRL_BEGIN(x, y, c, s)
@@ -69,9 +111,9 @@
         RG_CTRL_TICK(2);
         return iters;
     }
-    const float bgain = p.barrier_gain, ugain = p.unsafe_barrier_gain, qp_rtol = p.qp_rtol;
-    const int qp_cap = p.qp_max_sweeps;
-    const bool has_unsafe = p.barrier_has_unsafe_gain != 0;
+    const float bgain = k.bgain, ugain = k.ugain, qp_rtol = k.qp_rtol;
+    const int qp_cap = k.qp_cap;
+    const bool has_unsafe = k.has_unsafe != 0;
     float ex[GW - 1], ey[GW - 1], fx[GW - 1], fy[GW - 1], bp[GW - 1], emax[GW - 1];
     float mu[GW - 1], dmu[GW - 1];
     auto pair_consts = [&](float pxi, float pyi, int K, int i) {
@@ -220,9 +262,9 @@
     return my_sweeps;
 }
 
-template <int GW, int OD, int NT>
+template <int GW, int OD, int NT, typename Row>
 __device__ __forceinline__ void write_neighbour_obs(Lds<GW> &lds, int N, int Knb, int ag, int gbase, bool lane_ok,
-                                                    float x, float y, float *obs_row) {
+                                                    float x, float y, Row obs_row) {
     constexpr int M = NT > 0 ? NT - 1 : GW - 1;
     unsigned long long key[M > 0 ? M : 1];
     bool ok[M > 0 ? M : 1];
@@ -271,7 +313,7 @@
         const int j = who[r];
         const int slot = all_others ? (j < ag ? j : j - 1) : rank[r];
         if (ok[r] & (all_others | (slot < Knb))) {
-            float *o = obs_row + (slot + 1) * OD;
+            const auto o = obs_row + (slot + 1) * OD;
             if constexpr (OD == 4) {
                 out_store4(o, row[r][0], row[r][1], row[r][2], row[r][3]);
             } else {
@@ -291,17 +333,17 @@
     constexpr int EPW = WAVE / RW;
     RG_STAMPS_BEGIN()
     const rg_scenario_params &p = a.p;
-    const Consts &k = a.k;
     const float *q_poses = a.st.poses, *q_carry = a.st.carry_dist, *q_ret = a.st.ep_return, *q_sum = a.st.done_return_sum;
     const int32_t *q_steps = a.st.episode_steps, *q_act = sv.actions, *q_cnt = a.st.done_count, *q_stp = a.st.done_steps_sum;
     int32_t *q_el = GYM ? sv.io.elapsed : nullptr;
     const int q_tl = GYM ? sv.io.time_limit : 0;
     const int32_t *q_rc = a.st.reset_count, *q_nep = AHEAD ? a.st.next_episode : nullptr;
     const float *q_nin = AHEAD ? a.st.next_init : nullptr;
-    const int q_nst = AHEAD ? a.next_stride : 0;
-    const int q_E = a.E, q_epw = a.envs_per_wave, q_P = p.num_prey, q_N = p.n_agents, q_G = gridDim.x;
+    int q_nst = AHEAD ? a.next_stride : 0;
+    int q_auto = a.auto_reset;
+    int q_E = a.E, q_epw = a.envs_per_wave, q_P = p.num_prey, q_N = p.n_agents, q_G = gridDim.x;
     asm volatile("" ::"s"(q_poses), "s"(q_carry), "s"(q_ret), "s"(q_sum), "s"(q_steps), "s"(q_act), "s"(q_cnt), "s"(q_stp),
-                 "s"(q_E), "s"(q_epw), "s"(q_P), "s"(q_N), "s"(q_G), "s"(q_rc));
+                 "s"(q_E), "s"(q_epw), "s"(q_P), "s"(q_N), "s"(q_G), "s"(q_rc), "s"(q_auto));
     if constexpr (GYM) asm volatile("" ::"s"(q_el), "s"(q_tl));
     if constexpr (AHEAD) asm volatile("" ::"s"(q_nep), "s"(q_nin), "s"(q_nst));
     const float *q_prey = a.st.prey_loc;
@@ -313,6 +355,11 @@
     else if constexpr (SCN == RG_SCN_SIMPLE) asm volatile("" ::"s"(q_prey));
     else if constexpr (SCN == RG_SCN_ARCTIC_TRANSPORT) asm volatile("" ::"s"(q_grid), "s"(q_pix), "s"(q_reached), "s"(q_gcol));
     else asm volatile("" ::"s"(q_msg), "s"(q_zone), "s"(q_load));
+    constexpr bool PIN = QPM == 0;
+    if constexpr (PIN) {
+        asm volatile("" : "+s"(q_E), "+s"(q_epw), "+s"(q_P), "+s"(q_N), "+s"(q_G), "+s"(q_auto));
+        if constexpr (AHEAD) asm volatile("" : "+s"(q_nst));
+    }
     int32_t *q_tidx = TEAM ? tm->team_index : nullptr;
     const float *q_tstep = TEAM ? tm->agent_step : nullptr, *q_tsr = TEAM ? tm->sensing_radius : nullptr;
     const float *q_tcr = TEAM ? tm->capture_radius : nullptr;
@@ -377,7 +424,7 @@
         }
     }
     int rc_raw = -1;
-    const bool ahead = AHEAD && (!OBS_ONLY) && q_nst > 0 && a.auto_reset;
+    const bool ahead = AHEAD && (!OBS_ONLY) && q_nst > 0 && q_auto;
     int nx_tag = -2;
     float nx_pose[3] = {0.0f, 0.0f, 0.0f};
     float nx_a = 0.0f, nx_b = 0.0f;
@@ -408,7 +455,7 @@
     int el_raw = 0;
     if (env_ok) {
         steps_raw = q_steps[e];
-        if (!OBS_ONLY && a.auto_reset) rc_raw = q_rc[e];
+        if (!OBS_ONLY && q_auto) rc_raw = q_rc[e];
         if constexpr (GYM) el_raw = q_el[e];
         if (ahead) nx_tag = q_nep[e];
         if (stats && ag == 0) {
@@ -497,10 +544,97 @@
         if (lane_ok) load = q_load[eN + ag];
     }
 
+    StepConsts kc = {};
+    uint32_t *pk = nullptr;
+    enum { PK_POSES, PK_CARRY, PK_STEPS, PK_RET, PK_SUM, PK_CNT, PK_STP, PK_S0, PK_S1, PK_S2,
+           PK_OBS, PK_REW, PK_DIST, PK_DONE, PK_VIOL, PK_REM, PK_QPS, PK_ADDRS };
+    enum { PW_MAXSTEPS = 2 * PK_ADDRS, PW_D, PW_SHARED, PW_KNB, PW_AWARE, PW_RVIOL, PW_RTIME, PW_F0, PW_F1, PW_F2, PW_F3,
+           PW_TQ0, PW_END = PW_TQ0 + (SCN == RG_SCN_MATERIAL_TRANSPORT ? GW : 0) };
+    static_assert(PW_END <= WAVE, "one word per lane");
+    constexpr bool PARK = PIN && !OBS_ONLY;
+    auto scn_const = [&](int i) {
+        if constexpr (SCN == RG_SCN_PREDATOR_CAPTURE_PREY) return i == 0 ? p.sense_reward : p.capture_reward;
+        else if constexpr (SCN == RG_SCN_WAREHOUSE) return i == 0 ? p.goal_width : i == 1 ? p.load_reward : p.unload_reward;
+        else if constexpr (SCN == RG_SCN_MATERIAL_TRANSPORT)
+            return i == 0 ? p.end_goal_width : i == 1 ? p.zone1_radius : i == 2 ? p.load_multiplier : p.unload_multiplier;
+        else return 0.0f;
+    };
+    constexpr int SCN_CONSTS = SCN == RG_SCN_PREDATOR_CAPTURE_PREY ? 2 : SCN == RG_SCN_WAREHOUSE ? 3 : SCN == RG_SCN_MATERIAL_TRANSPORT ? 4 : 0;
+    if constexpr (!OBS_ONLY) {
+        static_cast<Consts &>(kc) = a.k;
+        kc.left = p.left, kc.right = p.right, kc.up = p.up, kc.down = p.down;
+        kc.penalize = p.penalize_violations, kc.U = p.update_frequency, kc.period = p.controller_period;
+        kc.bgain = p.barrier_gain, kc.ugain = p.unsafe_barrier_gain, kc.qp_rtol = p.qp_rtol;
+        kc.qp_cap = p.qp_max_sweeps, kc.has_unsafe = p.barrier_has_unsafe_gain;
+    }
+    if constexpr (PARK) {
+        int park = 0;
+        float *o_obs = sv.io.obs, *o_rew = sv.io.reward, *o_dist = sv.io.dist_travelled;
+        uint8_t *o_done = sv.io.done, *o_viol = sv.io.violation;
+        int32_t *o_rem = sv.io.remaining, *o_qps = sv.io.qp_sweeps;
+        const int o_max = p.max_episode_steps, o_D = p.obs_dim, o_shared = p.shared_reward, o_knb = p.num_neighbors, o_aware = p.capability_aware;
+        const float o_rviol = p.violation_reward, o_rtime = p.time_penalty;
+        float o_f[4] = {0.0f, 0.0f, 0.0f, 0.0f};
+        static_for<0, SCN_CONSTS>([&](auto II) { o_f[decltype(II)::value] = scn_const(decltype(II)::value); });
+        asm volatile("" ::"s"(o_obs), "s"(o_rew), "s"(o_dist), "s"(o_done), "s"(o_viol), "s"(o_rem), "s"(o_qps), "s"(o_max), "s"(o_D),
+                     "s"(o_shared), "s"(o_knb), "s"(o_aware), "s"(o_rviol), "s"(o_rtime), "s"(o_f[0]), "s"(o_f[1]), "s"(o_f[2]), "s"(o_f[3]));
+        asm volatile("" ::"s"(kc.left), "s"(kc.right), "s"(kc.up), "s"(kc.down), "s"(kc.penalize), "s"(kc.U), "s"(kc.period),
+                     "s"(kc.bgain), "s"(kc.ugain), "s"(kc.qp_rtol), "s"(kc.qp_cap), "s"(kc.has_unsafe));
+        asm volatile("" ::"s"(kc.dt), "s"(kc.pd), "s"(kc.inv_pd), "s"(kc.r2), "s"(kc.wlim), "s"(kc.vmax), "s"(kc.wmax), "s"(kc.pvl),
+                     "s"(kc.bml), "s"(kc.xmin), "s"(kc.xmax), "s"(kc.ymin), "s"(kc.ymax), "s"(kc.coll_off), "s"(kc.coll_lim2),
+                     "s"(kc.thr_pre), "s"(kc.lin_pre), "s"(kc.xc), "s"(kc.xh), "s"(kc.yc), "s"(kc.yh));
+        asm volatile("" : "+s"(kc.left), "+s"(kc.right), "+s"(kc.up), "+s"(kc.down), "+s"(kc.penalize), "+s"(kc.U), "+s"(kc.period),
+                     "+s"(kc.bgain), "+s"(kc.ugain), "+s"(kc.qp_rtol), "+s"(kc.qp_cap), "+s"(kc.has_unsafe));
+        asm volatile("" : "+s"(kc.dt), "+s"(kc.pd), "+s"(kc.inv_pd), "+s"(kc.r2), "+s"(kc.wlim), "+s"(kc.vmax), "+s"(kc.wmax), "+s"(kc.pvl),
+                     "+s"(kc.bml), "+s"(kc.xmin), "+s"(kc.xmax), "+s"(kc.ymin), "+s"(kc.ymax), "+s"(kc.coll_off), "+s"(kc.coll_lim2),
+                     "+s"(kc.thr_pre), "+s"(kc.lin_pre), "+s"(kc.xc), "+s"(kc.xh), "+s"(kc.yc), "+s"(kc.yh));
+        park_put<PK_POSES>(park, q_poses);
+        park_put<PK_CARRY>(park, q_carry);
+        park_put<PK_STEPS>(park, q_steps);
+        park_put<PK_RET>(park, q_ret);
+        park_put<PK_SUM>(park, q_sum);
+        park_put<PK_CNT>(park, q_cnt);
+        park_put<PK_STP>(park, q_stp);
+        if constexpr (SCN == RG_SCN_PREDATOR_CAPTURE_PREY) {
+            park_put<PK_S0>(park, q_sen);
+            park_put<PK_S1>(park, q_cap);
+        } else if constexpr (SCN == RG_SCN_WAREHOUSE) {
+            park_put<PK_S0>(park, q_loaded);
+        } else if constexpr (SCN == RG_SCN_MATERIAL_TRANSPORT) {
+            park_put<PK_S0>(park, q_load);
+            park_put<PK_S1>(park, q_zone);
+            park_put<PK_S2>(park, q_msg);
+        }
+        park_put<PK_OBS>(park, o_obs);
+        park_put<PK_REW>(park, o_rew);
+        park_put<PK_DIST>(park, o_dist);
+        park_put<PK_DONE>(park, o_done);
+        park_put<PK_VIOL>(park, o_viol);
+        park_put<PK_REM>(park, o_rem);
+        park_put<PK_QPS>(park, o_qps);
+        park_word<PW_MAXSTEPS>(park, o_max);
+        park_word<PW_D>(park, o_D);
+        park_word<PW_SHARED>(park, o_shared);
+        park_word<PW_KNB>(park, o_knb);
+        park_word<PW_AWARE>(park, o_aware);
+        park_word<PW_RVIOL>(park, __builtin_bit_cast(int, o_rviol));
+        park_word<PW_RTIME>(park, __builtin_bit_cast(int, o_rtime));
+        park_word<PW_F0>(park, __builtin_bit_cast(int, o_f[0]));
+        park_word<PW_F1>(park, __builtin_bit_cast(int, o_f[1]));
+        park_word<PW_F2>(park, __builtin_bit_cast(int, o_f[2]));
+        park_word<PW_F3>(park, __builtin_bit_cast(int, o_f[3]));
+        if constexpr (SCN == RG_SCN_MATERIAL_TRANSPORT && !TEAM)
+            static_for<0, GW>([&](auto JJ) { park_word<PW_TQ0 + decltype(JJ)::value>(park, p.torque[decltype(JJ)::value]); });
+        pk = park_lds();
+        pk[lane] = park;
+        park_publish();
+    }
+
     int viol = 0, max_sweeps = 0;
     bool replayed = false;
     float dist = 0.0f;
     if constexpr (!OBS_ONLY) {
+        const StepConsts &k = kc;
         RG_PIN5(x, y, th, carry, act);
         RG_STAMP(0);
         float gx = x, gy = y;
@@ -513,11 +647,11 @@
                 const float ice = pix == 1 ? fast_s : pix == 2 ? slow_s : nrm_s;
                 sd = ag < 2 ? fast_s : ag == 3 ? water : ice;
             }
-            const float cgx = clamp_spec(gx, p.left, p.right), cgy = clamp_spec(gy, p.up, p.down);
-            const float lft = (gx - sd) > p.left ? (gx - sd) : p.left;
-            const float rgt = (gx + sd) < p.right ? (gx + sd) : p.right;
-            const float upw = (gy - sd) > p.up ? (gy - sd) : p.up;
-            const float dwn = (gy + sd) < p.down ? (gy + sd) : p.down;
+            const float cgx = clamp_spec(gx, k.left, k.right), cgy = clamp_spec(gy, k.up, k.down);
+            const float lft = (gx - sd) > k.left ? (gx - sd) : k.left;
+            const float rgt = (gx + sd) < k.right ? (gx + sd) : k.right;
+            const float upw = (gy - sd) > k.up ? (gy - sd) : k.up;
+            const float dwn = (gy + sd) < k.down ? (gy + sd) : k.down;
             gx = mv == 0 ? lft : mv == 1 ? rgt : cgx;
             gy = mv == 2 ? upw : mv == 3 ? dwn : cgy;
         }
@@ -530,8 +664,8 @@
         bool dead = false;
         float fin_x = 0.0f, fin_y = 0.0f;
         float bx = x, by = y, ox = 0.0f, oy = 0.0f;
-        const bool penalize = p.penalize_violations != 0;
-        const int U = p.update_frequency, period = p.controller_period;
+        const bool penalize = k.penalize != 0;
+        const int U = k.U, period = k.period;
         for (int it0 = 0; it0 < U; it0 += period) {
             const int n = (U - it0) < period ? (U - it0) : period;
             RG_HEADING_SINCOS(th, s, c);
@@ -723,8 +857,34 @@
         RG_CHUNK_REPORT()
     }
 
-    const int D = p.obs_dim;
-    float *obs_row = sv.io.obs + (eN + ag) * D;
+    RG_SHADOW_SCALAR_TRIPS()
+    auto word = [&](auto LL, int direct) {
+        if constexpr (PARK) return static_cast<int>(pk[decltype(LL)::value]);
+        else return direct;
+    };
+    auto fword = [&](auto LL, float direct) {
+        if constexpr (PARK) return __builtin_bit_cast(float, pk[decltype(LL)::value]);
+        else return direct;
+    };
+    auto addr = [&](auto II, auto *direct) {
+        using T = std::remove_pointer_t<decltype(direct)>;
+        if constexpr (PARK) return park_get<T, decltype(II)::value>(pk);
+        else return (GlobalPtr<T>)direct;
+    };
+    auto uniform = [&](int v) { return PARK ? __builtin_amdgcn_readfirstlane(v) : v; };
+#define RG_PW(l) std::integral_constant<int, l> {}
+    const auto e_obs = addr(RG_PW(PK_OBS), sv.io.obs);
+    const int e_D = uniform(word(RG_PW(PW_D), p.obs_dim)), e_knb = word(RG_PW(PW_KNB), p.num_neighbors);
+    const int e_aware = uniform(word(RG_PW(PW_AWARE), p.capability_aware));
+    const int e_shared = uniform(word(RG_PW(PW_SHARED), p.shared_reward)), max_steps = word(RG_PW(PW_MAXSTEPS), p.max_episode_steps);
+    const float e_rviol = fword(RG_PW(PW_RVIOL), p.violation_reward), e_rtime = fword(RG_PW(PW_RTIME), p.time_penalty);
+    const float e_f0 = fword(RG_PW(PW_F0), scn_const(0)), e_f1 = fword(RG_PW(PW_F1), scn_const(1));
+    const float e_f2 = fword(RG_PW(PW_F2), scn_const(2)), e_f3 = fword(RG_PW(PW_F3), scn_const(3));
+    const float e_rsense = e_f0, e_rcapture = e_f1;
+    const float e_gw = e_f0, e_rload = e_f1, e_runload = e_f2;
+    const float e_egw = e_f0, e_z1r = e_f1, e_mload = e_f2, e_munload = e_f3;
+    const int D = e_D;
+    const auto obs_row = e_obs + (eN + ag) * D;
     bool done = false;
     int remaining = -1;
     float reward = 0.0f;
@@ -733,7 +893,7 @@
     RG_LATE(rc_raw);
     RG_LATE(nx_tag);
     const bool have_next = ahead & (nx_tag == rc_raw);
-    const bool next_early = env_ok & have_next & ((viol != 0) | (steps > p.max_episode_steps));
+    const bool next_early = env_ok & have_next & ((viol != 0) | (steps > max_steps));
     if constexpr (AHEAD) load_next(next_early & !helper);
 
     if constexpr (SCN == RG_SCN_PREDATOR_CAPTURE_PREY) {
@@ -792,14 +952,15 @@
                 c_b = group_or<GW>(c_b);
                 nsen_lo = sen_lo | (s_b & ~cap_lo);
                 ncap_lo = cap_lo | (nsen_lo & c_b & ~cap_lo);
+                const auto e_sen = addr(RG_PW(PK_S0), a.st.prey_sensed), e_cap = addr(RG_PW(PK_S1), a.st.prey_captured);
                 if (env_st && ag < P) {
-                    a.st.prey_sensed[static_cast<size_t>(e) * P + ag] = (nsen_lo >> ag) & 1u;
-                    a.st.prey_captured[static_cast<size_t>(e) * P + ag] = (ncap_lo >> ag) & 1u;
+                    e_sen[static_cast<size_t>(e) * P + ag] = (nsen_lo >> ag) & 1u;
+                    e_cap[static_cast<size_t>(e) * P + ag] = (ncap_lo >> ag) & 1u;
                 }
                 if constexpr (GW < 8)
                     if (env_ok && ag + GW < P) {
-                        a.st.prey_sensed[static_cast<size_t>(e) * P + ag + GW] = (nsen_lo >> (ag + GW)) & 1u;
-                        a.st.prey_captured[static_cast<size_t>(e) * P + ag + GW] = (ncap_lo >> (ag + GW)) & 1u;
+                        e_sen[static_cast<size_t>(e) * P + ag + GW] = (nsen_lo >> (ag + GW)) & 1u;
+                        e_cap[static_cast<size_t>(e) * P + ag + GW] = (ncap_lo >> (ag + GW)) & 1u;
                     }
             }
 #pragma unroll
@@ -833,12 +994,13 @@
                 nsen_hi = sen_hi | (s_hi & ~cap_hi);
                 ncap_hi = cap_hi | (nsen_hi & c_hi & ~cap_hi);
             }
+            const auto e_sen = addr(RG_PW(PK_S0), a.st.prey_sensed), e_cap = addr(RG_PW(PK_S1), a.st.prey_captured);
             if (env_st) {
                 for (int i = ag; i < P; i += GW) {
                     const uint32_t sw_ = i < 32 ? nsen_lo >> i : nsen_hi >> (i - 32);
                     const uint32_t cw_ = i < 32 ? ncap_lo >> i : ncap_hi >> (i - 32);
-                    a.st.prey_sensed[static_cast<size_t>(e) * P + i] = sw_ & 1u;
-                    a.st.prey_captured[static_cast<size_t>(e) * P + i] = cw_ & 1u;
+                    e_sen[static_cast<size_t>(e) * P + i] = sw_ & 1u;
+                    e_cap[static_cast<size_t>(e) * P + i] = cw_ & 1u;
                 }
             }
         }
@@ -857,7 +1019,7 @@
         }
         }
         RG_STAMP_E(0);
-        const int od = p.capability_aware ? 6 : 4;
+        const int od = e_aware ? 6 : 4;
         lds.own[lane][0] = x;
         lds.own[lane][1] = y;
         lds.own[lane][2] = qx;
@@ -870,10 +1032,10 @@
 #pragma unroll
                 for (int cc = 0; cc < 6; ++cc) obs_row[cc] = lds.own[lane][cc];
             }
-            write_neighbour_obs<GW, 6, NT>(lds, N, p.num_neighbors, ag, gbase, lane_st, x, y, obs_row);
+            write_neighbour_obs<GW, 6, NT>(lds, N, e_knb, ag, gbase, lane_st, x, y, obs_row);
         } else {
             if (lane_st) out_store4(obs_row, x, y, qx, qy);
-            write_neighbour_obs<GW, 4, NT>(lds, N, p.num_neighbors, ag, gbase, lane_st, x, y, obs_row);
+            write_neighbour_obs<GW, 4, NT>(lds, N, e_knb, ag, gbase, lane_st, x, y, obs_row);
         }
         RG_STAMP_E(1);
         if constexpr (!OBS_ONLY) {
@@ -882,14 +1044,14 @@
             const int unseen1 = P - __builtin_popcount(nsen_lo) - __builtin_popcount(nsen_hi);
             const int left1 = P - __builtin_popcount(ncap_lo) - __builtin_popcount(ncap_hi);
             if (viol) {
-                reward = p.violation_reward;
+                reward = e_rviol;
                 done = true;
             } else {
                 reward = 0.0f;
-                reward = reward + static_cast<float>(unseen0 - unseen1) * p.sense_reward;
-                reward = reward + static_cast<float>(left0 - left1) * p.capture_reward;
-                reward = reward + p.time_penalty;
-                if (steps > p.max_episode_steps || left1 == 0) {
+                reward = reward + static_cast<float>(unseen0 - unseen1) * e_rsense;
+                reward = reward + static_cast<float>(left0 - left1) * e_rcapture;
+                reward = reward + e_rtime;
+                if (steps > max_steps || left1 == 0) {
                     done = true;
                     remaining = left1;
                 }
@@ -905,26 +1067,26 @@
             obs_row[1] = y;
             obs_row[2] = loaded ? 1.0f : 0.0f;
         }
-        write_neighbour_obs<GW, 3, NT>(lds, N, p.num_neighbors, ag, gbase, lane_st, x, y, obs_row);
+        write_neighbour_obs<GW, 3, NT>(lds, N, e_knb, ag, gbase, lane_st, x, y, obs_row);
         if constexpr (!OBS_ONLY) {
             if (viol) {
-                reward = p.violation_reward;
+                reward = e_rviol;
                 done = true;
             } else {
                 const bool green = (ag % 2) == 0;
                 if (loaded) {
-                    if (x < -1.5f + p.goal_width && ((green && y > 0.0f) || (!green && y <= 0.0f))) {
-                        reward = p.unload_reward;
+                    if (x < -1.5f + e_gw && ((green && y > 0.0f) || (!green && y <= 0.0f))) {
+                        reward = e_runload;
                         loaded = 0;
                     }
                 } else {
-                    if (x > 1.5f - p.goal_width && ((!green && y > 0.0f) || (green && y <= 0.0f))) {
-                        reward = p.load_reward;
+                    if (x > 1.5f - e_gw && ((!green && y > 0.0f) || (green && y <= 0.0f))) {
+                        reward = e_rload;
                         loaded = 1;
                     }
                 }
-                done = steps > p.max_episode_steps;
-                if (lane_st) a.st.loaded[eN + ag] = static_cast<uint8_t>(loaded);
+                done = steps > max_steps;
+                if (lane_st) addr(RG_PW(PK_S0), a.st.loaded)[eN + ag] = static_cast<uint8_t>(loaded);
             }
         }
     } else if constexpr (SCN == RG_SCN_SIMPLE) {
@@ -946,7 +1108,7 @@
                 const float dx = x - goal_x, dy = y - goal_y;
                 const float r = -(dx * dx + dy * dy);
                 reward = r * p.reward_scaler;
-                done = steps > p.max_episode_steps;
+                done = steps > max_steps;
             }
         }
     } else if constexpr (SCN == RG_SCN_ARCTIC_TRANSPORT) {
@@ -992,7 +1154,7 @@
                 const int r_ = rc >> 4, c_ = rc & 15;
                 const int left = c_ > 0 ? c_ - 1 : c_, right = c_ < 11 ? c_ + 1 : c_;
                 const int up = r_ > 0 ? r_ - 1 : r_, down = r_ < 7 ? r_ + 1 : r_;
-                float *o = obs_row + 14 + 8 * i;
+                const auto o = obs_row + 14 + 8 * i;
                 o[0] = static_cast<float>(grid[up * 12 + left]);
                 o[1] = static_cast<float>(grid[r_ * 12 + left]);
                 o[2] = static_cast<float>(grid[down * 12 + left]);
@@ -1003,7 +1165,7 @@
                 o[7] = static_cast<float>(grid[down * 12 + right]);
             }
         }
-        if constexpr (LIDAR) write_lidar<SCN, GW, OBS_ONLY, Sync>(*lid, a, lds, lane, gbase, N, ag, lane_ok, x, y, th, obs_row);
+        if constexpr (LIDAR) write_lidar<SCN, GW, OBS_ONLY, Sync>(*lid, a, lds, lane, gbase, N, ag, lane_ok, x, y, th, (float *)obs_row);
         if constexpr (!OBS_ONLY) {
             const float dx = x - goalx, dy = y - goaly;
             lds.ax[lane] = dx * dx + dy * dy;
@@ -1023,7 +1185,7 @@
                     if ((pr >> 1) != 3) reward = reward + p.dist_multiplier * lds.ax[gbase + j];
                     all_reached = all_reached && rj;
                 }
-                done = steps > p.max_episode_steps;
+                done = steps > max_steps;
                 if (!done) done = all_reached;
             }
             if (lane_ok) {
@@ -1046,7 +1208,7 @@
             obs_row[4] = static_cast<float>(zone1);
 #pragma unroll
             for (int i = 0; i < 4; ++i) obs_row[5 + i] = static_cast<float>(msg[i]);
-            if (p.capability_aware) {
+            if (e_aware) {
                 if constexpr (TEAM) obs_row[9] = static_cast<float>(tq_raw);
                 else obs_row[9] = static_cast<float>(p.torque[ag]);
                 obs_row[10] = agent_step;
@@ -1059,22 +1221,23 @@
             if constexpr (TEAM) team_lds<SCN, GW>().torque[lane] = tq_raw;
             Sync::sync();
             if (viol) {
-                reward = p.violation_reward;
+                reward = e_rviol;
                 done = true;
             } else {
-                reward = p.time_penalty;
-                const float egw = p.end_goal_width;
-                const float zr2 = p.zone1_radius * p.zone1_radius;
+                reward = e_rtime;
+                const float egw = e_egw;
+                const float zr2 = e_z1r * e_z1r;
                 bool any_load = false;
                 for (int j = 0; j < N; ++j) {
                     const float jx = lds.ax[gbase + j], jy = lds.ay[gbase + j];
                     int jl = lds.aload[gbase + j];
                     int tq;
                     if constexpr (TEAM) tq = team_lds<SCN, GW>().torque[gbase + j];
+                    else if constexpr (PARK) tq = static_cast<int>(pk[PW_TQ0 + j]);
                     else tq = p.torque[j];
                     if (jl > 0) {
                         if (jx < -1.5f + egw) {
-                            reward = reward + static_cast<float>(jl) * p.unload_multiplier;
+                            reward = reward + static_cast<float>(jl) * e_munload;
                             jl = 0;
                         }
                     } else {
@@ -1086,7 +1249,7 @@
                                 jl = zone1;
                                 zone1 = 0;
                             }
-                            reward = reward + static_cast<float>(jl) * p.load_multiplier;
+                            reward = reward + static_cast<float>(jl) * e_mload;
                         } else if (jx * jx + jy * jy <= zr2) {
                             if (zone0 > tq) {
                                 jl = tq;
@@ -1095,13 +1258,13 @@
                                 jl = zone0;
                                 zone0 = 0;
                             }
-                            reward = reward + static_cast<float>(jl) * p.load_multiplier;
+                            reward = reward + static_cast<float>(jl) * e_mload;
                         }
                     }
                     if (j == ag) load = jl;
                     any_load = any_load || (jl != 0);
                 }
-                done = steps > p.max_episode_steps;
+                done = steps > max_steps;
                 if (!done) done = (zone0 == 0 && zone1 == 0 && !any_load);
             }
             int total = 0;
@@ -1111,16 +1274,18 @@
                 for (int j = 0; j < N; ++j) total += lds.aload[gbase + j];
             }
             if (done) remaining = zone0 + zone1 + total;
-            if (lane_st) a.st.load[eN + ag] = load;
+            const auto e_load = addr(RG_PW(PK_S0), a.st.load), e_zone = addr(RG_PW(PK_S1), a.st.zone_load);
+            const auto e_msg = addr(RG_PW(PK_S2), a.st.messages);
+            if (lane_st) e_load[eN + ag] = load;
             if (lane_st && ag == 0) {
-                a.st.zone_load[2 * e] = zone0;
-                a.st.zone_load[2 * e + 1] = zone1;
-            }
-            if (lane_st && ag < 4) a.st.messages[4 * e + ag] = msg[ag == 0 ? 0 : ag == 1 ? 1 : ag == 2 ? 2 : 3];
-        }
-    }
-
-    if constexpr (LIDAR && SCN != RG_SCN_ARCTIC_TRANSPORT) write_lidar<SCN, GW, OBS_ONLY, Sync>(*lid, a, lds, lane, gbase, N, ag, lane_ok, x, y, th, obs_row);
+                e_zone[2 * e] = zone0;
+                e_zone[2 * e + 1] = zone1;
+            }
+            if (lane_st && ag < 4) e_msg[4 * e + ag] = msg[ag == 0 ? 0 : ag == 1 ? 1 : ag == 2 ? 2 : 3];
+        }
+    }
+
+    if constexpr (LIDAR && SCN != RG_SCN_ARCTIC_TRANSPORT) write_lidar<SCN, GW, OBS_ONLY, Sync>(*lid, a, lds, lane, gbase, N, ag, lane_ok, x, y, th, (float *)obs_row);
     RG_STAMP(4);
     if constexpr (!OBS_ONLY) {
         constexpr bool gym = GYM;
@@ -1131,46 +1296,53 @@
         }
         const bool ended = done | trunc;
         float rsum = 0.0f;
-        if ((stats && !p.shared_reward) || gym) {
+        if ((stats && !e_shared) || gym) {
             Sync::sync();
             lds.ax[lane] = lane_ok ? reward : 0.0f;
             Sync::sync();
             for (int j = 0; j < N; ++j) rsum = rsum + lds.ax[gbase + j];
         }
+        const auto e_poses = addr(RG_PW(PK_POSES), a.st.poses), e_carry = addr(RG_PW(PK_CARRY), a.st.carry_dist);
+        const auto e_rew = addr(RG_PW(PK_REW), sv.io.reward), e_dist = addr(RG_PW(PK_DIST), sv.io.dist_travelled);
+        const auto e_done = addr(RG_PW(PK_DONE), sv.io.done), e_viol = addr(RG_PW(PK_VIOL), sv.io.violation);
+        const auto e_rem = addr(RG_PW(PK_REM), sv.io.remaining), e_qps = addr(RG_PW(PK_QPS), sv.io.qp_sweeps);
+        const auto e_steps = addr(RG_PW(PK_STEPS), a.st.episode_steps);
+        const auto e_ret = addr(RG_PW(PK_RET), a.st.ep_return), e_sum = addr(RG_PW(PK_SUM), a.st.done_return_sum);
+        const auto e_cnt = addr(RG_PW(PK_CNT), a.st.done_count), e_stp = addr(RG_PW(PK_STP), a.st.done_steps_sum);
         if (lane_st) {
-            float *X = a.st.poses + eN * 3;
+            const auto X = e_poses + eN * 3;
             X[ag] = x;
             X[N + ag] = y;
             X[2 * N + ag] = th;
-            a.st.carry_dist[eN + ag] = carry;
-            out_store1(sv.io.reward + eN + ag, reward);
-            out_store1(sv.io.dist_travelled + eN + ag, dist);
+            e_carry[eN + ag] = carry;
+            out_store1(e_rew + eN + ag, reward);
+            out_store1(e_dist + eN + ag, dist);
             if (ag == 0) {
-                a.st.episode_steps[e] = steps;
+                e_steps[e] = steps;
                 if (stats) {
                     RG_LATE(st_ret);
                     RG_LATE(st_sum);
                     RG_LATE(st_cnt);
                     RG_LATE(st_steps);
-                    float ret = st_ret + (p.shared_reward ? reward : rsum);
+                    float ret = st_ret + (e_shared ? reward : rsum);
                     if (ended) {
-                        a.st.done_return_sum[e] = st_sum + ret;
-                        a.st.done_count[e] = st_cnt + 1;
-                        a.st.done_steps_sum[e] = st_steps + steps;
+                        e_sum[e] = st_sum + ret;
+                        e_cnt[e] = st_cnt + 1;
+                        e_stp[e] = st_steps + steps;
                         ret = 0.0f;
                     }
-                    a.st.ep_return[e] = ret;
-                }
-                sv.io.done[e] = done ? 1 : 0;
+                    e_ret[e] = ret;
+                }
+                e_done[e] = done ? 1 : 0;
                 if (gym) {
                     q_el[e] = ended ? 0 : el_raw + 1;
                     sv.io.truncated[e] = trunc ? 1 : 0;
                     sv.io.ended[e] = ended ? 1 : 0;
                     sv.io.reward_sum[e] = rsum;
                 }
-                sv.io.violation[e] = static_cast<uint8_t>(viol);
-                sv.io.remaining[e] = remaining;
-                if (sv.io.qp_sweeps) sv.io.qp_sweeps[e] = max_sweeps;
+                e_viol[e] = static_cast<uint8_t>(viol);
+                e_rem[e] = remaining;
+                if (e_qps) e_qps[e] = max_sweeps;
             }
             if constexpr (GYM) {
                 if (sv.io.zero_obs_on_end && ended) {
@@ -1179,7 +1351,7 @@
             }
         }
         RG_STAMP(5);
-        if (a.auto_reset && __any(env_ok & ended)) {
+        if (q_auto && __any(env_ok & ended)) {
             Sync::sync();
             if constexpr (AHEAD) load_next(env_st & ended & have_next & !next_early);
             if (__any(env_ok & ended & !have_next)) reset_group<SCN, GW, Sync>(a, lds, e, g, ag, env_st & ended & !have_next, rc_raw);
@@ -1238,6 +1410,7 @@
         RG_STAMP(6);
         RG_STAMPS_WRITE(lane, sv.io.qp_sweeps, chunk * EPW, a.E, max_sweeps)
     }
+#undef RG_PW
 }
 
 template <int SCN, int GW, bool OBS_ONLY, int NT, bool ROLLOUT, bool GYM, int QPM, bool SPAN>
```

New measurement: 1.613 billion. 0.984x the previous value.
